# graehl/carmel

Hardware: AMD Instinct MI355X
Metric: arc-updates/sec (EM iterations/sec x derivation-lattice arcs swept per iteration) (higher is better)
Workload: dtype f64; 1 GPU; c4: synthetic 1000000-state / 9999990-arc WFST, 1000000 training pairs per GPU (random walks of 5-40 arcs), conditional normalisation, cached lattices; parallelism=corpus-sharded x1, none

## Files before the change

### carmel_amd/_capi.py

```python
import ctypes as C
import os

import numpy as np

_HERE = os.path.dirname(os.path.abspath(__file__))
LIB_PATH = os.environ.get("CARMEL_HIP_LIB") or os.path.join(_HERE, "libcarmel_hip.so")

SYMBOLS = [
    "carmel_hip_last_error", "carmel_hip_device_count", "carmel_hip_create", "carmel_hip_destroy",
    "carmel_hip_set_corpus", "carmel_hip_build_lattices", "carmel_hip_set_norm", "carmel_hip_set_prior",
    "carmel_hip_set_cascade", "carmel_hip_normalize", "carmel_hip_set_weights", "carmel_hip_get_weights",
    "carmel_hip_get_arc_weights", "carmel_hip_estimate", "carmel_hip_estimate_async",
    "carmel_hip_estimate_finish", "carmel_hip_counts_dev", "carmel_hip_counts_len", "carmel_hip_stream",
    "carmel_hip_use_external_counts", "carmel_hip_synchronize", "carmel_hip_last_sweep_ms", "carmel_hip_read_scalars",
    "carmel_hip_get_counts", "carmel_hip_set_counts", "carmel_hip_maximize", "carmel_hip_keep_em_weights", "carmel_hip_random_restart", "carmel_hip_save_counts",
    "carmel_hip_fractional_counts", "carmel_hip_set_digamma",
    "carmel_hip_save_best", "carmel_hip_load_best", "carmel_hip_host_build", "carmel_hip_host_dims",
    "carmel_hip_host_export", "carmel_hip_host_export_lanes", "carmel_hip_host_export_waves", "carmel_hip_host_transpose", "carmel_hip_host_tile_sweep", "carmel_hip_host_free",
    "carmel_hip_gibbs_create", "carmel_hip_gibbs_destroy", "carmel_hip_gibbs_n_blocks", "carmel_hip_gibbs_lattice_stats", "carmel_hip_gibbs_max_sample",
    "carmel_hip_gibbs_run", "carmel_hip_gibbs_run_ex", "carmel_hip_gibbs_set_prior_inference", "carmel_hip_gibbs_prior_trace",
    "carmel_hip_gibbs_n_prior_scales", "carmel_hip_gibbs_set_run_share", "carmel_hip_gibbs_best_stats", "carmel_hip_forests_set_prior_inference", "carmel_hip_forests_prior_trace", "carmel_hip_gibbs_get_sample", "carmel_hip_gibbs_set_observer", "carmel_hip_gibbs_current_probs", "carmel_hip_gibbs_get_state", "carmel_hip_gibbs_final_counts", "carmel_hip_gibbs_uniform", "carmel_hip_gibbs_power", "carmel_hip_gibbs_best_run", "carmel_hip_gibbs_set_init_weights",
    "carmel_hip_forests_create", "carmel_hip_forests_destroy", "carmel_hip_forests_estimate",
    "carmel_hip_forests_get_counts", "carmel_hip_forests_maximize", "carmel_hip_forests_get_weights",
    "carmel_hip_forests_set_weights", "carmel_hip_forests_set_alphas", "carmel_hip_forests_gibbs", "carmel_hip_forests_best_run", "carmel_hip_forests_final_counts", "carmel_hip_forests_get_sample",
    "carmel_hip_forests_max_sample", "carmel_hip_forests_viterbi", "carmel_hip_forests_get_viterbi",
    "carmel_hip_compose", "carmel_hip_composition_states", "carmel_hip_composition_arcs", "carmel_hip_composition_seconds",
    "carmel_hip_composition_export", "carmel_hip_composition_free",
    "carmel_hip_debug_lattice_fingerprint", "carmel_hip_lattice_layout", "carmel_hip_lattice_tile_sweep", "carmel_hip_lattice_fused_lanes", "carmel_hip_lattice_weight_source", "carmel_hip_accumulate_counts",
    "carmel_hip_comm_unique_id", "carmel_hip_comm_create", "carmel_hip_comm_destroy", "carmel_hip_comm_rank",
    "carmel_hip_comm_world", "carmel_hip_allreduce_counts", "carmel_hip_comm_allreduce_host",
    "carmel_hip_comm_abort", "carmel_hip_comm_transport_name", "carmel_hip_comm_create_custom", "carmel_hip_comm_set_sendrecv", "carmel_hip_comm_selftest", "carmel_hip_exchange_plan",
    "carmel_hip_exchange_info", "carmel_hip_exchange_measure", "carmel_hip_exchange_clear", "carmel_hip_set_layout_policy", "carmel_hip_set_matrix_fb",
    "carmel_hip_set_option", "carmel_hip_get_option", "carmel_hip_option_count", "carmel_hip_option_name",
    "carmel_hip_decoder_create", "carmel_hip_decoder_set_weights", "carmel_hip_decode", "carmel_hip_decoder_get_paths",
    "carmel_hip_decoder_last_ms", "carmel_hip_decoder_destroy",
    "carmel_hip_decode_kbest", "carmel_hip_decoder_kbest_size", "carmel_hip_decoder_get_kbest",
    "carmel_hip_decode_sum",
]


class LatticeStats(C.Structure):
    _fields_ = [(n, C.c_uint64) for n in (
        "n_pairs", "n_pairs_kept", "explored_states", "explored_arcs", "kept_states", "kept_arcs",
        "n_cyclic_pairs", "n_bundles", "max_levels", "device_bytes")] + [("build_seconds", C.c_double)] + [
            (n, C.c_uint64) for n in ("last_pair_explored_states", "last_pair_kept_states", "last_pair_kept_arcs",
                                      "n_windowed_pairs")]


class EstimateResult(C.Structure):
    _fields_ = [("sum_logprob", C.c_double), ("sum_weighted_logprob", C.c_double), ("n_pairs", C.c_uint64),
                ("kernel_ms", C.c_double)]


GIBBS_OBSERVER_FN = C.CFUNCTYPE(None, C.c_void_p, C.c_uint32, C.c_uint32, C.c_double)


class GibbsOpts(C.Structure):
    _fields_ = [("iter", C.c_uint32), ("burnin", C.c_uint32), ("seed", C.c_uint64), ("mode", C.c_int),
                ("uniform_p0", C.c_int), ("dirichlet_p0", C.c_int), ("final_counts", C.c_int),
                ("exclude_prior", C.c_int), ("min_prior", C.c_double), ("high_temp", C.c_double),
                ("low_temp", C.c_double), ("expectation", C.c_int), ("restarts", C.c_uint32), ("argmax_final", C.c_int),
                ("argmax_sum", C.c_int), ("include_self", C.c_int), ("random_start", C.c_int)]


def _load():
    if not os.path.exists(LIB_PATH):
        raise ImportError(
            "carmel_amd: %s not found — build it with `make -C carmel_amd/csrc` (or __graft_entry__.build()); "
            "there is no CPU fallback for the EM hot path" % LIB_PATH)
    lib = C.CDLL(LIB_PATH)
    for s in SYMBOLS:
        if not hasattr(lib, s):
            raise ImportError("carmel_amd: %s lacks symbol %s" % (LIB_PATH, s))
    lib.carmel_hip_last_error.restype = C.c_char_p
    lib.carmel_hip_counts_dev.restype = C.c_void_p
    lib.carmel_hip_stream.restype = C.c_void_p
    lib.carmel_hip_counts_len.restype = C.c_uint64
    vp = C.c_void_p
    lib.carmel_hip_last_error.argtypes = []
    lib.carmel_hip_device_count.argtypes = []
    lib.carmel_hip_set_option.argtypes = [C.c_char_p, C.c_char_p]
    lib.carmel_hip_get_option.argtypes = [C.c_char_p]
    lib.carmel_hip_get_option.restype = C.c_char_p
    lib.carmel_hip_option_count.argtypes = []
    lib.carmel_hip_option_name.argtypes = [C.c_int]
    lib.carmel_hip_option_name.restype = C.c_char_p
    lib.carmel_hip_random_restart.argtypes = [vp, C.c_uint64, C.c_uint32]
    lib.carmel_hip_keep_em_weights.argtypes = [vp]
    lib.carmel_hip_comm_unique_id.argtypes = [vp]
    lib.carmel_hip_debug_lattice_fingerprint.argtypes = [vp, vp]
    lib.carmel_hip_compose.argtypes = [C.POINTER(vp), C.c_int, C.c_uint32, vp, vp, vp, vp, vp, C.c_uint32, vp, vp, vp, vp, vp, vp,
                                       C.c_uint32, vp, C.c_uint32, C.c_uint32]
    lib.carmel_hip_composition_states.argtypes = [vp]
    lib.carmel_hip_composition_states.restype = C.c_uint64
    lib.carmel_hip_composition_arcs.argtypes = [vp]
    lib.carmel_hip_composition_arcs.restype = C.c_uint64
    lib.carmel_hip_composition_seconds.argtypes = [vp]
    lib.carmel_hip_composition_seconds.restype = C.c_double
    lib.carmel_hip_composition_export.argtypes = [vp] * 11
    lib.carmel_hip_composition_free.argtypes = [vp]
    lib.carmel_hip_comm_create.argtypes = [C.POINTER(vp), C.c_int, C.c_int, C.c_int, vp]
    lib.carmel_hip_comm_destroy.argtypes = [vp]
    lib.carmel_hip_comm_abort.argtypes = [vp]
    lib.carmel_hip_comm_transport_name.argtypes = [vp]
    lib.carmel_hip_comm_transport_name.restype = C.c_char_p
    lib.carmel_hip_comm_create_custom.argtypes = [C.POINTER(vp), C.c_int, C.c_int, C.c_int, vp]
    lib.carmel_hip_comm_set_sendrecv.argtypes = [vp, vp]
    lib.carmel_hip_comm_selftest.argtypes = [vp, C.c_uint32]
    lib.carmel_hip_exchange_plan.argtypes = [vp, vp, C.c_uint32, C.c_int]
    lib.carmel_hip_exchange_info.argtypes = [vp, C.POINTER(C.c_int), C.POINTER(C.c_uint32), C.POINTER(C.c_uint64), C.POINTER(C.c_uint64),
                                             C.POINTER(C.c_uint64)]
    lib.carmel_hip_exchange_measure.argtypes = [vp, C.c_uint32, C.POINTER(C.c_double)]
    lib.carmel_hip_exchange_clear.argtypes = [vp]
    lib.carmel_hip_set_layout_policy.argtypes = [vp, C.c_int]
    lib.carmel_hip_set_matrix_fb.argtypes = [vp, C.c_int]
    lib.carmel_hip_comm_rank.argtypes = [vp]
    lib.carmel_hip_comm_world.argtypes = [vp]
    lib.carmel_hip_allreduce_counts.argtypes = [vp, vp]
    lib.carmel_hip_comm_allreduce_host.argtypes = [vp, vp, C.c_uint32, C.c_int]
    lib.carmel_hip_fractional_counts.argtypes = [vp]
    lib.carmel_hip_set_digamma.argtypes = [vp, C.c_uint32, vp, vp]
    lib.carmel_hip_forests_set_alphas.argtypes = [vp, vp, C.c_uint32]
    lib.carmel_hip_create.argtypes = [C.POINTER(vp), C.c_int, C.c_uint32, C.c_uint32, C.c_uint64, vp, vp, vp, vp, vp, vp]
    lib.carmel_hip_destroy.argtypes = [vp]
    lib.carmel_hip_set_corpus.argtypes = [vp, C.c_uint64, vp, vp, vp, vp, vp]
    lib.carmel_hip_build_lattices.argtypes = [vp, C.c_int, C.c_int, vp, C.POINTER(LatticeStats)]
    lib.carmel_hip_set_norm.argtypes = [vp, C.c_int, C.c_double]
    lib.carmel_hip_set_prior.argtypes = [vp, C.c_double, C.c_int]
    lib.carmel_hip_set_cascade.argtypes = [vp, C.c_uint64, vp, vp, vp, vp, vp, C.c_uint32, vp, vp, C.c_uint64, vp, vp]
    lib.carmel_hip_normalize.argtypes = [vp]
    lib.carmel_hip_set_weights.argtypes = [vp, vp]
    lib.carmel_hip_get_weights.argtypes = [vp, vp]
    lib.carmel_hip_get_arc_weights.argtypes = [vp, vp]
    lib.carmel_hip_estimate.argtypes = [vp, C.POINTER(EstimateResult), vp]
    lib.carmel_hip_estimate_async.argtypes = [vp]
    lib.carmel_hip_estimate_finish.argtypes = [vp, C.POINTER(EstimateResult), vp]
    lib.carmel_hip_counts_dev.argtypes = [vp]
    lib.carmel_hip_counts_len.argtypes = [vp]
    lib.carmel_hip_stream.argtypes = [vp]
    lib.carmel_hip_use_external_counts.argtypes = [vp, vp]
    lib.carmel_hip_synchronize.argtypes = [vp]
    lib.carmel_hip_last_sweep_ms.argtypes = [vp, C.POINTER(C.c_double)]
    lib.carmel_hip_read_scalars.argtypes = [vp, C.POINTER(EstimateResult)]
    lib.carmel_hip_get_counts.argtypes = [vp, vp]
    lib.carmel_hip_set_counts.argtypes = [vp, vp]
    lib.carmel_hip_maximize.argtypes = [vp, C.c_double, C.POINTER(C.c_double)]
    lib.carmel_hip_save_counts.argtypes = [vp]
    lib.carmel_hip_save_best.argtypes = [vp]
    lib.carmel_hip_load_best.argtypes = [vp]
    lib.carmel_hip_host_build.argtypes = [C.POINTER(vp), C.c_uint32, C.c_uint32, C.c_uint64, vp, vp, vp, vp,
                                          C.c_uint64, vp, vp, vp, vp, vp, C.c_int, C.c_int, C.c_uint32, C.c_uint32,
                                          C.c_int]
    lib.carmel_hip_host_dims.argtypes = [vp, vp]
    lib.carmel_hip_host_dims.restype = None
    lib.carmel_hip_host_export.argtypes = [vp] + [vp] * 12
    lib.carmel_hip_host_export.restype = None
    lib.carmel_hip_host_export_lanes.argtypes = [vp] * 8
    lib.carmel_hip_host_export_waves.argtypes = [vp] * 10
    lib.carmel_hip_host_transpose.argtypes = [vp] * 12
    lib.carmel_hip_host_transpose.restype = None
    lib.carmel_hip_host_tile_sweep.argtypes = [vp] * 3
    lib.carmel_hip_host_tile_sweep.restype = None
    lib.carmel_hip_host_export_lanes.restype = None
    lib.carmel_hip_host_free.argtypes = [vp]
    lib.carmel_hip_host_free.restype = None
    lib.carmel_hip_gibbs_create.argtypes = [C.POINTER(vp), vp, C.POINTER(GibbsOpts)]
    lib.carmel_hip_gibbs_destroy.argtypes = [vp]
    lib.carmel_hip_gibbs_n_blocks.argtypes = [vp]
    lib.carmel_hip_gibbs_lattice_stats.argtypes = [vp, C.POINTER(LatticeStats)]
    lib.carmel_hip_gibbs_n_blocks.restype = C.c_uint32
    lib.carmel_hip_gibbs_max_sample.argtypes = [vp]
    lib.carmel_hip_gibbs_max_sample.restype = C.c_uint32
    lib.carmel_hip_gibbs_set_init_weights.argtypes = [vp, vp]
    lib.carmel_hip_gibbs_best_run.argtypes = [vp]
    lib.carmel_hip_gibbs_best_run.restype = C.c_uint32
    lib.carmel_hip_gibbs_run.argtypes = [vp, vp, vp]
    lib.carmel_hip_gibbs_run_ex.argtypes = [vp, vp, vp, vp]
    lib.carmel_hip_gibbs_set_prior_inference.argtypes = [vp, C.c_double, C.c_int, C.c_int, C.c_int, C.c_uint32, C.c_uint32, vp, vp, C.c_uint32]
    lib.carmel_hip_gibbs_prior_trace.argtypes = [vp, vp, C.c_uint32, vp, C.c_uint32]
    lib.carmel_hip_gibbs_n_prior_scales.argtypes = [vp]
    lib.carmel_hip_gibbs_set_run_share.argtypes = [vp, C.c_uint32, C.c_uint32]
    lib.carmel_hip_gibbs_best_stats.argtypes = [vp, vp, vp]
    lib.carmel_hip_lattice_layout.argtypes = [vp]
    lib.carmel_hip_lattice_tile_sweep.argtypes = [vp]
    lib.carmel_hip_lattice_fused_lanes.argtypes = [vp]
    lib.carmel_hip_lattice_weight_source.argtypes = [vp]
    lib.carmel_hip_accumulate_counts.argtypes = [vp, C.c_int]
    lib.carmel_hip_forests_set_prior_inference.argtypes = [vp, C.c_double, C.c_int, C.c_int, C.c_uint32, C.c_uint32]
    lib.carmel_hip_forests_prior_trace.argtypes = [vp, vp, C.c_uint32, vp, C.c_uint32, vp]
    lib.carmel_hip_gibbs_n_prior_scales.restype = C.c_uint32
    lib.carmel_hip_gibbs_get_sample.argtypes = [vp, C.c_uint32, vp, C.POINTER(C.c_uint32)]
    lib.carmel_hip_gibbs_set_observer.argtypes = [vp, C.c_uint32, GIBBS_OBSERVER_FN, vp]
    lib.carmel_hip_gibbs_current_probs.argtypes = [vp, vp]
    lib.carmel_hip_gibbs_get_state.argtypes = [vp, vp, vp, vp, vp, vp]
    lib.carmel_hip_gibbs_final_counts.argtypes = [vp, vp]
    lib.carmel_hip_gibbs_uniform.argtypes = [C.c_uint64, C.c_uint32, C.c_uint32, C.c_uint32]
    lib.carmel_hip_gibbs_uniform.restype = C.c_double
    lib.carmel_hip_gibbs_power.argtypes = [C.c_double, C.c_double, C.c_uint32, C.c_uint32]
    lib.carmel_hip_gibbs_power.restype = C.c_double
    lib.carmel_hip_forests_create.argtypes = [C.POINTER(vp), C.c_int, C.c_uint64, vp, vp, vp, vp, C.c_uint32, vp,
                                              C.c_uint64, vp, vp]
    lib.carmel_hip_forests_destroy.argtypes = [vp]
    lib.carmel_hip_forests_estimate.argtypes = [vp, C.c_double, C.POINTER(C.c_double), C.POINTER(C.c_uint64), vp]
    lib.carmel_hip_forests_get_counts.argtypes = [vp, C.c_double, vp]
    lib.carmel_hip_forests_maximize.argtypes = [vp, C.c_double, C.c_double, C.c_int, C.POINTER(C.c_double)]
    lib.carmel_hip_forests_get_weights.argtypes = [vp, vp]
    lib.carmel_hip_forests_set_weights.argtypes = [vp, vp]
    lib.carmel_hip_forests_gibbs.argtypes = [vp, C.POINTER(GibbsOpts), C.c_double, vp, vp]
    lib.carmel_hip_forests_best_run.argtypes = [vp]
    lib.carmel_hip_forests_best_run.restype = C.c_uint32
    lib.carmel_hip_forests_final_counts.argtypes = [vp, vp]
    lib.carmel_hip_forests_get_sample.argtypes = [vp, C.c_uint64, vp, C.POINTER(C.c_uint32)]
    lib.carmel_hip_forests_max_sample.argtypes = [vp]
    lib.carmel_hip_forests_max_sample.restype = C.c_uint32
    lib.carmel_hip_forests_viterbi.argtypes = [vp, vp]
    lib.carmel_hip_forests_get_viterbi.argtypes = [vp, C.c_uint64, vp, vp, C.POINTER(C.c_uint32)]
    lib.carmel_hip_decoder_create.argtypes = [C.POINTER(vp), C.c_int, C.c_uint32, C.c_uint32, C.c_uint64, vp, vp, vp, vp, vp,
                                              C.c_int]
    lib.carmel_hip_decoder_set_weights.argtypes = [vp, vp]
    lib.carmel_hip_decode.argtypes = [vp, C.c_uint64, vp, vp, vp, vp]
    lib.carmel_hip_decoder_get_paths.argtypes = [vp, vp]
    lib.carmel_hip_decoder_last_ms.argtypes = [vp, C.POINTER(C.c_double)]
    lib.carmel_hip_decoder_destroy.argtypes = [vp]
    lib.carmel_hip_decode_kbest.argtypes = [vp, C.c_uint32, C.c_uint64, vp, vp, vp]
    lib.carmel_hip_decoder_kbest_size.argtypes = [vp, C.POINTER(C.c_uint64), C.POINTER(C.c_uint64)]
    lib.carmel_hip_decoder_get_kbest.argtypes = [vp, vp, vp, vp]
    lib.carmel_hip_decode_sum.argtypes = [vp, C.c_uint64, vp, vp, vp]
    for s in SYMBOLS:
        if getattr(lib, s).argtypes is None:
            raise ImportError("carmel_amd: no ctypes prototype for %s" % s)
    return lib


lib = _load()


class CarmelHipError(RuntimeError):
    def __init__(self, code, where):
        self.code = code
        RuntimeError.__init__(self, "%s failed (%d): %s" % (where, code, lib.carmel_hip_last_error().decode()))


def check(rc, where):
    if rc != 0:
        raise CarmelHipError(rc, where)


def set_option(key, value):
    rc = lib.carmel_hip_set_option(key.encode(), None if value is None else str(value).encode())
    if rc != 0:
        raise ValueError("libcarmel_hip has no option %r (it has: %s)" % (key, ", ".join(option_names())))


def get_option(key):
    v = lib.carmel_hip_get_option(key.encode())
    return None if v is None else v.decode()


def option_names():
    return [lib.carmel_hip_option_name(i).decode() for i in range(lib.carmel_hip_option_count())]


def options_from_env(environ=None):
    names = set(option_names())
    for k, v in (os.environ if environ is None else environ).items():
        key = "timing" if k == "CARMEL_TIMING" else k[len("CARMEL_HIP_"):].lower() if k.startswith("CARMEL_HIP_") and k != "CARMEL_HIP_LIB" else None
        if key in names:
            set_option(key, v)


def ptr(a):
    if a is None:
        return None
    assert a.flags["C_CONTIGUOUS"]
    return a.ctypes.data_as(C.c_void_p)


def u32(a):
    return np.ascontiguousarray(a, dtype=np.uint32)


def u64(a):
    return np.ascontiguousarray(a, dtype=np.uint64)


def f64(a):
    return np.ascontiguousarray(a, dtype=np.float64)
```

### carmel_amd/csrc/engine.cpp

```cpp
#include <hip/hip_runtime.h>
#include <chrono>
#include <cmath>
#include <cstdio>
#include <cstring>
#include <cstdlib>
#include <limits>
#include <string>
#include <thread>
#include <unordered_map>
#include <vector>
#include "engine.hpp"
#include "options.hpp"
#include "host/refhash.hpp"
#include "rng.hpp"
#include "unrolled_args.hpp"

int unrolled_try_build(carmel_hip_trainer* t, int host_threads, uint8_t* has_derivation, carmel_hip_lattice_stats* stats);
int gpu_build_lattices(carmel_hip_trainer* t, const BuildOptions& opt, uint8_t* has_derivation, carmel_hip_lattice_stats* stats,
                       bool& done);
int gpu_tables_for_host_layout(carmel_hip_trainer* t, const std::vector<uint32_t>& lane_arc, const std::vector<uint32_t>& wave_arc);
int carmel_hip_debug_lattice_fingerprint_impl(carmel_hip_trainer* t, uint64_t* out);
int build_run_tables(carmel_hip_trainer* t);
int exchange_weights_in(carmel_hip_trainer* t, ExchangePlan* xp, const TransArgs& T, bool need_x);
int exchange_counts_out(carmel_hip_trainer* t, ExchangePlan* xp, const TransArgs& T);
int exchange_counts_tail(carmel_hip_trainer* t, ExchangePlan* xp);
int exchange_maximize(carmel_hip_trainer* t, ExchangePlan* xp, double* max_change, int* handled);
int exchange_settle(carmel_hip_trainer* t, bool need_counts);
void exchange_drop(carmel_hip_trainer* t);
int unrolled_estimate(carmel_hip_trainer* t, hipStream_t s);

static thread_local std::string g_err;
namespace carmel_hip {
int fail(int code, const std::string& msg) {
  g_err = msg;
  return code;
}
}

template <class F>
static void host_parallel_for(size_t n, F f) {
  const size_t nt = n < (1u << 20) ? 1 : std::min<size_t>(16, std::max<unsigned>(1, std::thread::hardware_concurrency()));
  if (nt <= 1) {
    f(0, n);
    return;
  }
  std::vector<std::thread> th;
  for (size_t k = 0; k < nt; ++k) th.emplace_back([&, k]() { f(n * k / nt, n * (k + 1) / nt); });
  for (auto& x : th) x.join();
}

extern "C" {

const char* carmel_hip_last_error(void) { return g_err.c_str(); }

int carmel_hip_device_count(void) {
  int n = 0;
  if (hipGetDeviceCount(&n) != hipSuccess) return 0;
  return n;
}

int carmel_hip_create(carmel_hip_trainer** out, int device, uint32_t n_states, uint32_t final_state, uint64_t n_arcs,
                      const uint32_t* src, const uint32_t* dst, const uint32_t* in_sym, const uint32_t* out_sym,
                      const double* logw, const uint32_t* group) {
  if (!out || !src || !dst || !in_sym || !out_sym || !logw) return fail(CARMEL_HIP_ERR_ARG, "null argument");
  if (final_state >= n_states) return fail(CARMEL_HIP_ERR_ARG, "final state out of range");
  if (n_arcs >= 0xfffffff0ull) return fail(CARMEL_HIP_ERR_ARG, "arc ids are 32-bit (derivations.h GraphArc data)");
  int ndev = 0;
  HIPCHK(hipGetDeviceCount(&ndev));
  if (ndev <= 0) return fail(CARMEL_HIP_ERR_HIP, "no HIP device: the EM hot path has no CPU fallback");
  if (device < 0 || device >= ndev) return fail(CARMEL_HIP_ERR_ARG, "bad device index");
  HIPCHK(hipSetDevice(device));
  carmel_hip_trainer* t = new carmel_hip_trainer();
  t->device = device;
  hipError_t e = hipStreamCreateWithFlags(&t->stream, hipStreamNonBlocking);
  if (e != hipSuccess) {
    delete t;
    return fail(CARMEL_HIP_ERR_HIP, hipGetErrorString(e));
  }
  (void)hipEventCreate(&t->ev0);
  (void)hipEventCreate(&t->ev1);
  (void)hipStreamCreateWithFlags(&t->side, hipStreamNonBlocking);
  (void)hipEventCreateWithFlags(&t->ev_fork, hipEventDisableTiming);
  (void)hipEventCreateWithFlags(&t->ev_join, hipEventDisableTiming);
  (void)hipEventCreateWithFlags(&t->ev_w, hipEventDisableTiming);
  if (hipHostMalloc((void**)&t->h_box, 2 * sizeof(unsigned long long), hipHostMallocCoherent | hipHostMallocMapped) != hipSuccess) t->h_box = nullptr;
  if (t->h_box) t->h_box[0] = t->h_box[1] = 0;
  (void)hipStreamCreateWithFlags(&t->bstream, hipStreamNonBlocking);
  (void)hipEventCreateWithFlags(&t->ev_b0, hipEventDisableTiming);
  (void)hipEventCreateWithFlags(&t->ev_b1, hipEventDisableTiming);
  for (int k = 0; k < carmel_hip_trainer::N_CHUNK_STREAMS; ++k) {
    (void)hipStreamCreateWithFlags(&t->cstream[k], hipStreamNonBlocking);
    (void)hipEventCreateWithFlags(&t->cev[k], hipEventDisableTiming);
  }
  HostWfst& w = t->w;
  w.n_states = n_states;
  w.final_state = final_state;
  w.n_arcs = n_arcs;
  w.src.assign(src, src + n_arcs);
  w.dst.assign(dst, dst + n_arcs);
  w.in.assign(in_sym, in_sym + n_arcs);
  w.out.assign(out_sym, out_sym + n_arcs);
  if (group)
    w.group.assign(group, group + n_arcs);
  else
    w.group.assign(n_arcs, CARMEL_HIP_NO_GROUP);
  for (uint64_t k = 0; k < n_arcs; ++k) {
    if (src[k] >= n_states || dst[k] >= n_states) {
      delete t;
      return fail(CARMEL_HIP_ERR_ARG, "arc endpoint out of range");
    }
    if (k && src[k] < src[k - 1]) {
      delete t;
      return fail(CARMEL_HIP_ERR_ARG, "arcs must be in arc-id order (state-major)");
    }
  }
  w.build_index();
  std::vector<double> lw(logw, logw + n_arcs);
  e = t->arc_logw.upload(lw, t->stream);
  if (e == hipSuccess) e = t->arc_group.upload(w.group, t->stream);
  if (e == hipSuccess) e = t->counts.alloc(n_arcs + 4);
  if (e == hipSuccess) e = t->old_logw.alloc(n_arcs);
  if (e == hipSuccess) e = t->em_logw.alloc(n_arcs);
  if (e == hipSuccess) e = t->best_logw.alloc(n_arcs);
  if (e == hipSuccess) e = t->maxchg.alloc(1);
  if (e == hipSuccess) e = hipStreamSynchronize(t->stream);
  if (e != hipSuccess) {
    delete t;
    return fail(CARMEL_HIP_ERR_HIP, hipGetErrorString(e));
  }
  *out = t;
  return CARMEL_HIP_OK;
}

int carmel_hip_destroy(carmel_hip_trainer* t) {
  if (t && t->xplan) exchange_drop(t);
  if (!t) return CARMEL_HIP_OK;
  (void)hipSetDevice(t->device);
  if (t->stream) (void)hipStreamSynchronize(t->stream);
  if (t->matrix) matrix_release(t->matrix);
  t->matrix = nullptr;
  if (t->ev0) (void)hipEventDestroy(t->ev0);
  if (t->ev1) (void)hipEventDestroy(t->ev1);
  if (t->side) (void)hipStreamSynchronize(t->side);
  if (t->ev_fork) (void)hipEventDestroy(t->ev_fork);
  if (t->ev_join) (void)hipEventDestroy(t->ev_join);
  if (t->ev_w) (void)hipEventDestroy(t->ev_w);
  if (t->h_box) (void)hipHostFree(t->h_box);
  if (t->bstream) {
    (void)hipStreamSynchronize(t->bstream);
    (void)hipStreamDestroy(t->bstream);
  }
  if (t->ev_b0) (void)hipEventDestroy(t->ev_b0);
  if (t->ev_b1) (void)hipEventDestroy(t->ev_b1);
  for (int k = 0; k < carmel_hip_trainer::N_CHUNK_STREAMS; ++k) {
    if (t->cstream[k]) {
      (void)hipStreamSynchronize(t->cstream[k]);
      (void)hipStreamDestroy(t->cstream[k]);
    }
    if (t->cev[k]) (void)hipEventDestroy(t->cev[k]);
    if (k == 0) {
      for (hipEvent_t e : t->ev_piece)
        if (e) (void)hipEventDestroy(e);
      t->ev_piece.clear();
    }
  }
// ... 17 lines not shown
    c.weight.assign(pair_weight, pair_weight + n_pairs);
  else
    c.weight.assign(n_pairs, 1.0);
  t->have_corpus = true;
  t->have_lattices = false;
  return CARMEL_HIP_OK;
}

int carmel_hip_build_lattices(carmel_hip_trainer* t, int prune, int host_threads, uint8_t* has_derivation,
                              carmel_hip_lattice_stats* stats) {
  if (!t) return fail(CARMEL_HIP_ERR_ARG, "null trainer");
  if (!t->have_corpus) return fail(CARMEL_HIP_ERR_STATE, "set_corpus first");
  HIPCHK(hipSetDevice(t->device));
  if (t->xplan) exchange_drop(t);
  if (t->scalars_pending) {
    (void)hipStreamSynchronize(t->side);
    t->scalars_pending = false;
  }
  t->build_prune = prune;
  t->build_threads = host_threads;
  if (t->matrix) {
    HIPCHK(hipStreamSynchronize(t->stream));
    matrix_release(t->matrix);
    t->matrix = nullptr;
  }
  {
    int rc = unrolled_try_build(t, host_threads, has_derivation, stats);
    if (rc) return rc;
    if (t->unrolled) return CARMEL_HIP_OK;
  }
  auto t0 = std::chrono::steady_clock::now();
  BuildOptions opt;
  opt.prune = prune != 0;
  opt.threads = host_threads;
  if (const char* e = lib_opt("lane_states")) opt.lane_states = (uint32_t)atoi(e);
  if (const char* e = lib_opt("tile_sweep")) opt.tile_sweep = atoi(e) != 0;
  if (const char* e = lib_opt("lane_fused")) opt.lane_fused = atoi(e) != 0;
  if (lib_opt("transpose") && atoi(lib_opt("transpose")) == 0) opt.lane_fused = false;
  if (const char* e = lib_opt("lane_chunks")) opt.lane_chunks = (uint32_t)std::max(1, atoi(e));
  if (const char* e = lib_opt("lane_window")) opt.lane_window = (uint32_t)std::max(0, atoi(e));
  if (const char* e = lib_opt("lane_window_min")) opt.lane_window_min = (uint32_t)std::max(0, atoi(e));
  if (const char* e = lib_opt("wave_ring")) opt.wave_ring = atoi(e) != 0;
  if (const char* e = lib_opt("wave_min_width")) opt.wave_min_width = opt.wave_lane_min_width = atof(e);
  {
    const bool want_gpu = !(lib_opt("gpu_build") && atoi(lib_opt("gpu_build")) == 0) &&
                          !(lib_opt("transpose") && atoi(lib_opt("transpose")) == 0);
    bool probe_ok = true;
    if (want_gpu && t->corpus.n_pairs > 4096) {
      const uint64_t np = t->corpus.n_pairs, n_probe = 64;
      for (uint64_t k = 0; k < n_probe && probe_ok; ++k) {
        const uint64_t p = k * (np / n_probe);
        PairLattice pl;
        bool hd = false;
        build_pair_lattice(t->w, t->corpus.in_sym.data() + t->corpus.in_off[p], (uint32_t)(t->corpus.in_off[p + 1] - t->corpus.in_off[p]),
                           t->corpus.out_sym.data() + t->corpus.out_off[p], (uint32_t)(t->corpus.out_off[p + 1] - t->corpus.out_off[p]),
                           opt.prune, pl, hd);
        if (pl.explored_states > 200 || (hd && (pl.n_states > opt.lane_states || pl.edges.size() > 200))) opt.gpu_large_caps = true;
        if (pl.explored_states > 1024 || (hd && (pl.cyclic || pl.n_states > 1023 || pl.edges.size() > 1536))) probe_ok = false;
      }
    }
    if (want_gpu && probe_ok) {
      bool done = false;
      int rc = gpu_build_lattices(t, opt, has_derivation, stats, done);
      if (rc) return rc;
      if (!done && !opt.gpu_large_caps) {
        opt.gpu_large_caps = true;
        rc = gpu_build_lattices(t, opt, has_derivation, stats, done);
        if (rc) return rc;
        if (!done) opt.gpu_large_caps = false;
      }
      if (done) {
        if (lib_opt("timing")) fprintf(stderr, "timing: lattices built on the GPU\n");
        rc = build_run_tables(t);
        if (stats) stats->device_bytes = t->device_bytes;
        return rc;
      }
    }
  }
  std::string err;
  LatticeSet& L = t->lat;
  L = LatticeSet();
  {
    const char* e = lib_opt("wave_gather");
    const bool want_t = !(lib_opt("transpose") && atoi(lib_opt("transpose")) == 0);
    opt.wave_gather = want_t && (e ? atoi(e) != 0 : t->w.n_arcs * sizeof(double) <= (128ull << 20));
  }
  opt.device_tables = !(lib_opt("transpose") && atoi(lib_opt("transpose")) == 0) &&
                      !(lib_opt("device_tables") && atoi(lib_opt("device_tables")) == 0);
  if (!build_lattices(t->w, t->corpus, opt, L, err)) return fail(CARMEL_HIP_ERR_ARG, err);
  const bool have_tables = !L.t_buckets.empty() || L.tables_deferred;
  if (has_derivation) std::memcpy(has_derivation, L.has_deriv.data(), L.has_deriv.size());
  hipStream_t s = t->stream;
  HIPCHK(t->bundles.upload(L.bundles, s));
  HIPCHK(t->in_arcs.upload(L.in_arcs, s));
  HIPCHK(t->out_arcs.upload(L.out_arcs, s));
  HIPCHK(t->in_off.upload(L.in_off, s));
  HIPCHK(t->out_off.upload(L.out_off, s));
  HIPCHK(t->level_off.upload(L.level_off, s));
  HIPCHK(t->pair_start.upload(L.pair_start, s));
  HIPCHK(t->pair_final.upload(L.pair_final, s));
  HIPCHK(t->pair_id.upload(L.pair_id, s));
  HIPCHK(t->pair_logw.upload(L.pair_logw, s));
  HIPCHK(t->lane_groups.upload(L.lane_groups, s));
  if (L.tile_sweep)
    HIPCHK(t->tile_group.upload(L.tile_group, s));
  else
    t->tile_group.release();
  HIPCHK(t->wave_descs.upload(L.waves, s));
  HIPCHK(t->wave_fwd.upload(L.wave_fwd, s));
  HIPCHK(t->wave_bwd.upload(L.wave_bwd, s));
  if (L.wave_gather && !L.waves.empty())
    HIPCHK(t->wave_bwd_arc.upload(L.wave_bwd_arc, s));
  else
    t->wave_bwd_arc.release();
  HIPCHK(t->wave_level_off.upload(L.wave_level_off, s));
  HIPCHK(t->wave_frow.upload(L.wave_frow, s));
  HIPCHK(t->wave_brow.upload(L.wave_brow, s));
  t->wave_slot_base = L.wave_slot_base;
  t->wave_records = L.wave_bwd.size();
  HIPCHK(t->wave_spill.alloc(L.wave_spill_states));
  {
    const bool want_t = !(lib_opt("transpose") && atoi(lib_opt("transpose")) == 0);
    if (want_t && have_tables) {
      std::vector<uint32_t> fx(L.lane_fwd.size());
      host_parallel_for(fx.size(), [&](size_t k0, size_t k1) {
        for (size_t k = k0; k < k1; ++k) fx[k] = L.lane_fwd[k].x;
      });
      HIPCHK(t->lane_fwdx.upload(fx, s));
      HIPCHK(hipStreamSynchronize(s));
      t->lane_fwd.release();
    } else {
      HIPCHK(t->lane_fwd.upload(L.lane_fwd, s));
      t->lane_fwdx.release();
    }
  }
  {
    std::vector<uint32_t> bx(L.lane_bwd.size());
    host_parallel_for(bx.size(), [&](size_t k0, size_t k1) {
      for (size_t k = k0; k < k1; ++k) bx[k] = L.lane_bwd[k].x;
    });
    HIPCHK(t->lane_bwd.upload(bx, s));
    HIPCHK(hipStreamSynchronize(s));
  }
  HIPCHK(t->lane_pair.upload(L.lane_pair, s));
  HIPCHK(t->lane_nstates.upload(L.lane_nstates, s));
  HIPCHK(t->lane_logw.upload(L.lane_logw, s));
  if (L.tile_sweep && t->lane_fwdx.n) {
    HIPCHK(t->lane_rec2.alloc(t->lane_bwd.n));
    HIPCHK(t->lane_chain.alloc(t->lane_groups.n));
    HIPCHK(t->tile_chain.alloc(t->tile_group.n - 1));
    HIPCHK(hipMemsetAsync(t->lane_rec2.p, 0, t->lane_rec2.bytes(), s));
    HIPCHK(launch_pack_tile_records(t->lane_groups.p, (uint32_t)t->lane_groups.n, t->lane_nstates.p, t->lane_fwdx.p, t->lane_bwd.p, t->lane_rec2.p, t->lane_chain.p,
                                    t->tile_group.p, (uint32_t)(t->tile_group.n - 1), t->tile_chain.p, s));
    if (lib_opt("timing")) {
      std::vector<uint32_t> ch(t->lane_chain.n);
      HIPCHK(hipMemcpyAsync(ch.data(), t->lane_chain.p, ch.size() * 4, hipMemcpyDeviceToHost, s));
      HIPCHK(hipStreamSynchronize(s));
      size_t n1 = 0;
      for (uint32_t c : ch) n1 += c & 1u;
      fprintf(stderr, "timing: tile sweep: %zu tiles, %zu groups, %zu of them single paths\n", L.tile_group.size() - 1, ch.size(), n1);
    }
  } else {
    t->lane_rec2.release();
    t->lane_chain.release();
    t->tile_chain.release();
  }
  t->lane_records = L.wave_slot_base + L.wave_bwd.size();
  if (L.lane_fused)
    t->post.release();
  else
    HIPCHK(t->post.alloc(L.n_post));
  HIPCHK(t->wcache.alloc(t->wave_bwd_arc.n ? L.wave_slot_base : t->lane_records));
  if (!L.waves.empty() && !have_tables)
    return fail(CARMEL_HIP_ERR_UNSUPPORTED, "lattice set too large for the blocked transposition (2^32 items) with one-per-wavefront lattices");
  if (L.lane_spill_rows)
    HIPCHK(t->lane_spill.alloc(L.lane_spill_rows * 64));
  else
    t->lane_spill.release();
  if (L.tables_deferred) {
    std::vector<uint32_t> la(L.lane_bwd.size());
    host_parallel_for(la.size(), [&](size_t k0, size_t k1) {
      for (size_t k = k0; k < k1; ++k) la[k] = (L.lane_bwd[k].x & LANE_VALID) ? L.lane_bwd[k].y : 0xffffffffu;
    });
    t->hot_chunks.release();
    int rc = gpu_tables_for_host_layout(t, la, L.wave_bwd_arc);
    if (rc) return rc;
    t->use_transpose = true;
  } else {
    HIPCHK(t->arc_off.upload(L.arc_off, s));
    HIPCHK(t->slot_pos.upload(L.slot_pos, s));
    HIPCHK(t->hot_chunks.upload(L.hot_chunks, s));
    {
      const bool want = !(lib_opt("transpose") && atoi(lib_opt("transpose")) == 0);
      t->use_transpose = want && !L.t_buckets.empty();
      if (t->use_transpose) {
        HIPCHK(t->t_buckets.upload(L.t_buckets, s));
        HIPCHK(t->t_tile_base.upload(L.t_tile_base, s));
        HIPCHK(t->t_b_arc.upload(L.t_b_arc, s));
        HIPCHK(t->t_b_rank.upload(L.t_b_rank, s));
        HIPCHK(t->t_b_src.upload(L.t_b_src, s));
        HIPCHK(t->t_t_pos.upload(L.t_t_pos, s));
        HIPCHK(t->t_t_src.upload(L.t_t_src, s));
        HIPCHK(t->t_a_off.upload(L.t_a_off, s));
        HIPCHK(t->t_split_arcs.upload(L.t_split_arcs, s));
        HIPCHK(t->t_x.alloc(L.slot_pos.size()));
        HIPCHK(t->t_xc.alloc(L.slot_pos.size()));
        HIPCHK(hipStreamSynchronize(s));
      }
      std::vector<uint16_t>().swap(L.t_b_arc);
      std::vector<uint16_t>().swap(L.t_a_off);
      std::vector<uint16_t>().swap(L.t_b_rank);
      std::vector<uint16_t>().swap(L.t_t_pos);
      std::vector<uint32_t>().swap(L.t_b_src);
      std::vector<uint32_t>().swap(L.t_t_src);
    }
  }
  if (!L.waves.empty() && !t->use_transpose)
    return fail(CARMEL_HIP_ERR_UNSUPPORTED, "one-per-wavefront lattices need the blocked transposition (CARMEL_HIP_TRANSPOSE=0 is for lane corpora)");
  HIPCHK(t->pair_logprob.alloc(t->corpus.n_pairs));
  {
    std::vector<double> pw(t->corpus.n_pairs);
    for (uint64_t p = 0; p < t->corpus.n_pairs; ++p)
      pw[p] = L.has_deriv[p] ? (t->corpus.weight.empty() ? 1.0 : t->corpus.weight[p]) : -1.0;
    HIPCHK(t->pair_w.upload(pw, s));
    HIPCHK(t->scalar_partial.alloc(3 * 256));
    HIPCHK(hipStreamSynchronize(s));
  }
  bool need_val = false, need_val2 = false;
  for (auto& lc : L.classes) {
    if (lc.serial || lc.max_states == 0) need_val = true;
    if (lc.serial) need_val2 = true;
  }
  HIPCHK(t->alpha_g.alloc(need_val ? L.in_off.size() : 0));
  HIPCHK(t->beta_g.alloc(need_val2 ? L.in_off.size() : 0));
  HIPCHK(launch_fill(t->pair_logprob.p, -std::numeric_limits<double>::infinity(), t->corpus.n_pairs, s));
  HIPCHK(hipStreamSynchronize(s));
  t->device_bytes = t->bundles.bytes() + t->in_arcs.bytes() + t->out_arcs.bytes() + t->in_off.bytes() +
                    t->out_off.bytes() + t->level_off.bytes() + t->pair_start.bytes() + t->pair_final.bytes() +
                    t->pair_id.bytes() + t->pair_logw.bytes() + t->pair_logprob.bytes() + t->alpha_g.bytes() +
                    t->beta_g.bytes() + t->lane_groups.bytes() + t->lane_fwd.bytes() + t->lane_fwdx.bytes() + t->lane_bwd.bytes() +
                    t->lane_pair.bytes() + t->lane_nstates.bytes() + t->lane_logw.bytes() + t->post.bytes() + t->wcache.bytes() +
                    t->arc_off.bytes() + t->slot_pos.bytes() + t->hot_chunks.bytes() + t->t_b_arc.bytes() + t->t_b_rank.bytes() +
                    t->t_t_pos.bytes() + t->t_b_src.bytes() + t->t_t_src.bytes() + t->t_x.bytes() + t->t_xc.bytes() +
                    t->wave_descs.bytes() + t->wave_fwd.bytes() + t->wave_bwd.bytes() + t->wave_bwd_arc.bytes() + t->wave_level_off.bytes() +
                    t->wave_frow.bytes() + t->wave_brow.bytes() + t->wave_spill.bytes();
  std::vector<uint64_t>().swap(L.arc_off);
  std::vector<uint64_t>().swap(L.slot_pos);
  std::vector<uint2_t>().swap(L.lane_fwd);
  std::vector<uint2_t>().swap(L.lane_bwd);
  std::vector<uint2_t>().swap(L.wave_fwd);
  std::vector<uint32_t>().swap(L.wave_bwd);
  std::vector<uint32_t>().swap(L.wave_bwd_arc);
  std::vector<uint2_t>().swap(L.in_arcs);
  std::vector<uint2_t>().swap(L.out_arcs);
  std::vector<uint32_t>().swap(L.in_off);
  std::vector<uint32_t>().swap(L.out_off);
  std::vector<uint32_t>().swap(L.level_off);
  if (lib_opt("timing")) {
    fprintf(stderr, "timing: layout lane_arcs=%llu lane_groups=%zu lane_pieces=%zu bundles=%zu bundle_classes=%zu total_arcs=%llu aligned=%d\n",
            (unsigned long long)L.lane_arcs, L.lane_groups.size(), L.lane_classes.size(), L.bundles.size(), L.classes.size(),
            (unsigned long long)L.total_arcs, (int)L.lane_tiles_aligned);
    for (auto& lc : L.lane_classes) fprintf(stderr, "timing:   lane piece groups=%u %s=%u tiles=%u\n", lc.count, lc.windowed ? "window" : "max_states", lc.max_states, lc.tile_count);
    for (auto& wc : L.wave_classes) fprintf(stderr, "timing:   wave class count=%u max_states=%u max_width=%u ring=%u\n", wc.count, wc.max_states, wc.max_width, wc.ring);
    for (auto& lc : L.classes) fprintf(stderr, "timing:   bundle class count=%u block=%u max_states=%u serial=%d\n", lc.count, lc.block, lc.max_states, (int)lc.serial);
  }
  t->have_lattices = true;
  ++t->lattice_epoch;
  {
    int rc = build_run_tables(t);
    if (rc) return rc;
  }
  if (stats) {
    stats->n_pairs = t->corpus.n_pairs;
    stats->n_pairs_kept = L.n_kept;
    stats->explored_states = L.explored_states;
    stats->explored_arcs = L.explored_arcs;
    stats->kept_states = L.total_states;
    stats->kept_arcs = L.total_arcs;
    stats->n_cyclic_pairs = L.n_cyclic;
    stats->n_bundles = L.bundles.size() + L.lane_groups.size() + L.waves.size();
    stats->max_levels = L.max_levels;
    stats->device_bytes = t->device_bytes;
    stats->build_seconds = std::chrono::duration<double>(std::chrono::steady_clock::now() - t0).count();
    stats->last_pair_explored_states = L.last_pre_states;
    stats->last_pair_kept_states = L.last_post_states;
    stats->last_pair_kept_arcs = L.last_post_arcs;
    stats->n_windowed_pairs = 0;
    for (auto& g : L.lane_groups)
      if (g.window) stats->n_windowed_pairs += g.n_lanes;
  }
  return CARMEL_HIP_OK;
}

static int build_ties(carmel_hip_trainer* t, uint64_t n, const uint32_t* member, const uint32_t* group) {
  std::vector<uint32_t> tie_of(n, 0xffffffffu);
  std::unordered_map<uint64_t, uint32_t> ids;
  t->any_locked = false;
  t->h_tie_member.clear();
  for (uint64_t k = 0; k < n; ++k) {
    if (group[k] == CARMEL_HIP_LOCKED_GROUP) t->any_locked = true;
    if (group[k] == CARMEL_HIP_NO_GROUP || group[k] == CARMEL_HIP_LOCKED_GROUP) continue;
    const uint64_t key = ((uint64_t)(member ? member[k] : 0) << 32) | group[k];
    auto it = ids.find(key);
    if (it == ids.end()) {
      it = ids.emplace(key, (uint32_t)ids.size()).first;
      t->h_tie_member.push_back(member ? member[k] : 0);
    }
    tie_of[k] = it->second;
  }
  t->n_ties = ids.size();
  if (t->n_ties) {
    HIPCHK(t->tie_of.upload(tie_of, t->stream));
    HIPCHK(t->tie_tab.alloc(4 * t->n_ties));
    HIPCHK(hipStreamSynchronize(t->stream));
  } else {
    t->tie_of.release();
    t->tie_tab.release();
  }
// ... 488 lines not shown
  A.out_arcs = (const uint2*)t->out_arcs.p;
  A.in_off = t->in_off.p;
  A.out_off = t->out_off.p;
  A.level_off = t->level_off.p;
  A.pair_start = t->pair_start.p;
  A.pair_final = t->pair_final.p;
  A.pair_id = t->pair_id.p;
  A.pair_logw = t->pair_logw.p;
  A.logw = t->arc_logw.p;
  A.post = t->post.p + t->lane_records;
  A.scalars = t->counts_ptr() + t->w.n_arcs;
  A.pair_logprob = t->pair_logprob.p;
  A.val_g = t->alpha_g.p;
  A.val2_g = t->beta_g.p;
  A.first_bundle = 0;
  LaneArgs LA;
  LA.groups = t->lane_groups.p;
  LA.fwd = (const uint2*)t->lane_fwd.p;
  LA.fwdx = t->lane_fwdx.p;
  LA.bwd = t->lane_bwd.p;
  LA.rec2 = t->lane_rec2.p;
  LA.chain = t->lane_chain.p;
  LA.tile_chain = t->tile_chain.p;
  LA.lane_pair = t->lane_pair.p;
  LA.lane_nstates = t->lane_nstates.p;
  LA.lane_logw = t->lane_logw.p;
  LA.logw = t->arc_logw.p;
  LA.post = t->post.p;
  LA.wcache = t->wcache.p;
  LA.scalars = t->counts_ptr() + t->w.n_arcs;
  LA.pair_logprob = t->pair_logprob.p;
  LA.spill = t->lane_spill.p;
  LA.first_group = 0;
  LA.lds_rows = 0;
  LA.xc_tile_base = nullptr;
  LA.xc_t_pos = nullptr;
  LA.xc = nullptr;
  LA.trace = nullptr;
  const char* trace_path = lib_opt("lane_trace");
  static DevBuf<unsigned long long> trace_buf;
  if (trace_path) {
    if (trace_buf.n != t->lane_groups.n * 16) {
      HIPCHK(trace_buf.alloc(t->lane_groups.n * 16));
      HIPCHK(hipMemset(trace_buf.p, 0, trace_buf.bytes()));
    }
    LA.trace = trace_buf.p;
  }
  WaveArgs WA;
  WA.descs = t->wave_descs.p;
  WA.fwd = (const uint2*)t->wave_fwd.p;
  WA.bwd = t->wave_bwd.p;
  WA.level_off = t->wave_level_off.p;
  WA.frow = t->wave_frow.p;
  WA.brow = t->wave_brow.p;
  WA.wcache = t->wcache.p + t->wave_slot_base;
  if (t->wave_bwd_arc.n) {
    WA.wcache = nullptr;
    WA.logw = t->arc_logw.p;
    WA.bwd_arc = t->wave_bwd_arc.p;
    WA.n_arcs = (uint32_t)t->w.n_arcs;
  }
  WA.post = t->post.p + t->wave_slot_base;
  WA.pair_logprob = t->pair_logprob.p;
  WA.spill = t->wave_spill.p;
  WA.first = 0;
  WA.max_states = WA.max_width = 0;
  TransArgs T;
  trans_args(t, T);
  const bool wave_xc = t->use_transpose && t->wave_xc_idx.n && !T.use_runs && !(T.scatter & 2u);
  if (wave_xc) {
    WA.xc = T.xc;
    WA.xc_idx = t->wave_xc_idx.p;
  }
  LA.pre_weights = t->use_transpose ? 1u : 0u;
  const bool lane_fused = t->use_transpose && t->lat.lane_fused &&
                          !(lib_opt("lane_fused_kernel") && atoi(lib_opt("lane_fused_kernel")) == 0);
  if (lane_fused) {
    LA.xc_tile_base = T.tile_base;
    LA.xc_t_pos = T.t_pos;
    LA.xc = T.xc;
  } else if (t->lat.lane_fused && !t->post.n && t->lat.n_post) {
    HIPCHK(t->post.alloc(t->lat.n_post));
    T.post = LA.post = t->post.p;
    T.n_post = t->post.n;
  }
  ExchangePlan* const xp = (t->xplan && exchange_is_sharded(t->xplan) && t->use_transpose) ? t->xplan : nullptr;
  if (timed) HIPCHK(hipEventRecord(t->ev0, s));
  const uint32_t lane_tiles = (uint32_t)((t->wcache.n + t->lat.tile - 1) / t->lat.tile);
  const bool tile_kernel_off = lib_opt("tile_sweep_kernel") && atoi(lib_opt("tile_sweep_kernel")) == 0;
  const bool tile_sweep = t->use_transpose && t->lat.tile_sweep && t->tile_group.n && !tile_kernel_off &&
                          ((T.scatter & 3u) == 0u || ((T.scatter & 3u) == 3u && T.use_runs));
  bool tile_sweep_done = false;
  const bool tile_gather = t->use_transpose && t->t_t_arc.n && !T.use_runs && !(T.scatter & 1u);
  TransArgs TW = T;
  if (tile_gather) {
    TW.x = const_cast<double*>(T.logw);
    TW.t_src = t->t_t_arc.p;
  }
  TransArgs TZ = TW;
  if (!xp) {
    TZ.zero_list = t->t_split_arcs.p;
    TZ.n_zero = (uint32_t)t->t_split_arcs.n;
  }
  const bool side_by_side = t->use_transpose && t->lat.lane_classes.size() > 1 && t->lat.lane_tiles_aligned && t->lat.wave_classes.empty();
  const bool bundles_beside = side_by_side && !t->lat.classes.empty();
  if (xp) {
    int rc = exchange_weights_in(t, xp, T, t->wcache.n && !tile_gather);
    if (rc) return rc;
  } else if (t->use_transpose && t->wcache.n && !tile_gather)
    HIPCHK(launch_trans_w_bucket(T, s));
  if (bundles_beside) {
    HIPCHK(hipEventRecord(t->ev_b0, s));
    HIPCHK(hipStreamWaitEvent(t->bstream, t->ev_b0, 0));
    for (auto& lc : t->lat.classes) HIPCHK(launch_sweep(A, lc, t->bstream));
    HIPCHK(hipEventRecord(t->ev_b1, t->bstream));
  }
  if (side_by_side && t->lat.lane_fused) {
    HIPCHK(hipEventRecord(t->ev_w, s));
    hipStream_t ps = t->side, ss = s;
    HIPCHK(hipStreamWaitEvent(ps, t->ev_w, 0));
    const size_t np = t->lat.lane_classes.size();
    while (t->ev_piece.size() < np) {
      hipEvent_t e = nullptr;
      HIPCHK(hipEventCreateWithFlags(&e, hipEventDisableTiming));
      t->ev_piece.push_back(e);
    }
    for (size_t k = 0; k < np; ++k) {
      const auto& lc = t->lat.lane_classes[k];
      HIPCHK(launch_trans_w_tiles(TW, lc.tile_first, lc.tile_count, ps));
      HIPCHK(hipEventRecord(t->ev_piece[k], ps));
      HIPCHK(hipStreamWaitEvent(ss, t->ev_piece[k], 0));
      HIPCHK(launch_lane_sweep(LA, lc, ss, lane_fused));
      if (!lane_fused) HIPCHK(launch_trans_c_tiles(T, lc.tile_first, lc.tile_count, ss));
    }
  } else if (side_by_side) {
    HIPCHK(hipEventRecord(t->ev_w, s));
    const int NS = carmel_hip_trainer::N_CHUNK_STREAMS;
    bool used[carmel_hip_trainer::N_CHUNK_STREAMS] = {false, false, false, false};
    size_t k = 0;
    for (auto& lc : t->lat.lane_classes) {
      hipStream_t cs = t->cstream[k % NS];
      if (!used[k % NS]) HIPCHK(hipStreamWaitEvent(cs, t->ev_w, 0));
      used[k % NS] = true;
      HIPCHK(launch_trans_w_tiles(TW, lc.tile_first, lc.tile_count, cs));
      HIPCHK(launch_lane_sweep(LA, lc, cs, lane_fused));
      if (!lane_fused) HIPCHK(launch_trans_c_tiles(T, lc.tile_first, lc.tile_count, cs));
      ++k;
    }
    for (int q = 0; q < NS; ++q)
      if (used[q]) {
        HIPCHK(hipEventRecord(t->cev[q], t->cstream[q]));
        HIPCHK(hipStreamWaitEvent(s, t->cev[q], 0));
      }
  } else if (tile_sweep && launch_tile_sweep(TZ, LA, t->tile_group.p, 0, lane_tiles, s) == hipSuccess) {
    tile_sweep_done = true;
  } else {
    if (tile_sweep) (void)hipGetLastError();
    if (t->use_transpose) HIPCHK(launch_trans_w_tiles(TW, 0, lane_tiles, s));
    if (t->lat.wave_classes.size() > 1 || (!t->lat.wave_classes.empty() && !t->lat.lane_classes.empty())) {
      HIPCHK(hipEventRecord(t->ev_w, s));
      const int NS = carmel_hip_trainer::N_CHUNK_STREAMS;
      bool used[carmel_hip_trainer::N_CHUNK_STREAMS] = {false, false, false, false};
      size_t k = 0;
      for (auto& wc : t->lat.wave_classes) {
        hipStream_t cs = t->cstream[k % NS];
        if (!used[k % NS]) HIPCHK(hipStreamWaitEvent(cs, t->ev_w, 0));
        used[k % NS] = true;
        HIPCHK(launch_wave_sweep(WA, wc, cs));
        ++k;
      }
      for (auto& lc : t->lat.lane_classes) HIPCHK(launch_lane_sweep(LA, lc, s, lane_fused));
      for (int q = 0; q < NS; ++q)
        if (used[q]) {
          HIPCHK(hipEventRecord(t->cev[q], t->cstream[q]));
          HIPCHK(hipStreamWaitEvent(s, t->cev[q], 0));
        }
    } else {
      for (auto& wc : t->lat.wave_classes) HIPCHK(launch_wave_sweep(WA, wc, s));
      for (auto& lc : t->lat.lane_classes) HIPCHK(launch_lane_sweep(LA, lc, s, lane_fused));
    }
  }
  if (bundles_beside)
    HIPCHK(hipStreamWaitEvent(s, t->ev_b1, 0));
  else
    for (auto& lc : t->lat.classes) HIPCHK(launch_sweep(A, lc, s));
  ReduceArgs R;
  R.arc_off = t->arc_off.p;
  R.slot_pos = t->slot_pos.p;
  R.hot_chunks = t->hot_chunks.p;
  R.post = t->post.p;
  R.counts = t->counts_ptr();
  R.n_arcs = t->w.n_arcs;
  R.n_hot_chunks = t->hot_chunks.n / 3;
  auto fork_scalars = [&](hipEvent_t fork) -> int {
    HIPCHK(hipEventRecord(fork, s));
    HIPCHK(hipStreamWaitEvent(t->side, fork, 0));
    HIPCHK(launch_scalars(t->pair_logprob.p, t->pair_w.p, t->corpus.n_pairs, t->scalar_partial.p,
                          t->counts_ptr() + t->w.n_arcs, t->side));
    HIPCHK(hipEventRecord(t->ev_join, t->side));
    t->scalars_pending = true;
    return CARMEL_HIP_OK;
  };
  if (xp) {
    int rc = fork_scalars(t->ev_fork);
    if (rc) return rc;
  }
  if (t->use_transpose) {
    const uint32_t first = (side_by_side || tile_sweep_done || lane_fused) ? lane_tiles : 0u;
    const uint32_t end = wave_xc ? std::min(T.n_tiles, (uint32_t)(t->wave_slot_base / t->lat.tile)) : T.n_tiles;
    HIPCHK(launch_trans_c_tiles(T, first, end > first ? end - first : 0u, s));
    if (xp) {
      int rc = exchange_counts_out(t, xp, T);
      if (rc) return rc;
    } else if (tile_sweep_done)
      HIPCHK(launch_trans_c_bucket_range(T, 0, T.n_buckets, s));
    else
      HIPCHK(launch_trans_c_bucket(T, t->t_split_arcs.p, (uint32_t)t->t_split_arcs.n, s));
  } else
    HIPCHK(launch_count_reduce(R, s));
  if (xp) {
    if (timed) HIPCHK(hipEventRecord(t->ev1, s));
  } else {
    int rc = fork_scalars(timed ? t->ev1 : t->ev_fork);
    if (rc) return rc;
  }
  if (xp || t->ext_counts) {
    int rc = scalars_join(t);
    if (rc) return rc;
  }
  if (xp) {
    int rc = exchange_counts_tail(t, xp);
    if (rc) return rc;
  }
  if (timed && trace_path && trace_buf.n) {
    std::vector<unsigned long long> h(trace_buf.n);
    HIPCHK(hipStreamSynchronize(s));
    HIPCHK(hipMemcpy(h.data(), trace_buf.p, h.size() * 8, hipMemcpyDeviceToHost));
    if (FILE* f = fopen(trace_path, "wb")) {
      fwrite(h.data(), 8, h.size(), f);
      fclose(f);
    }
  }
  return CARMEL_HIP_OK;
}

int carmel_hip_estimate_async(carmel_hip_trainer* t) {
  if (!t) return fail(CARMEL_HIP_ERR_ARG, "null trainer");
  if (!t->have_lattices) return fail(CARMEL_HIP_ERR_STATE, "build_lattices first");
  HIPCHK(hipSetDevice(t->device));
  return estimate_enqueue(t, true);
}

int carmel_hip_set_layout_policy(carmel_hip_trainer* t, int allow_unrolled) {
  if (!t) return fail(CARMEL_HIP_ERR_ARG, "null trainer");
  t->allow_unrolled = allow_unrolled != 0;
  return CARMEL_HIP_OK;
}
int carmel_hip_set_matrix_fb(carmel_hip_trainer* t, int on) {
  if (!t) return fail(CARMEL_HIP_ERR_ARG, "null trainer");
  HIPCHK(hipSetDevice(t->device));
  if (t->matrix) {
    HIPCHK(hipStreamSynchronize(t->stream));
    matrix_release(t->matrix);
    t->matrix = nullptr;
  }
  if (!on) return CARMEL_HIP_OK;
  if (!t->have_lattices) return fail(CARMEL_HIP_ERR_STATE, "carmel_hip_set_matrix_fb: build_lattices first (it finds the pairs without a derivation)");
  if (t->xplan) return fail(CARMEL_HIP_ERR_STATE, "carmel_hip_set_matrix_fb: drop the exchange plan first (the matrix E-step keeps the one all-reduce)");
  if (t->unrolled) {
    const bool keep = t->allow_unrolled;
    t->allow_unrolled = false;
    const int rc = carmel_hip_build_lattices(t, t->build_prune, t->build_threads, nullptr, nullptr);
    t->allow_unrolled = keep;
    if (rc) return rc;
  }
  return matrix_setup(t, &t->matrix);
}
int carmel_hip_lattice_tile_sweep(carmel_hip_trainer* t) {
  if (!t || !t->have_lattices || t->unrolled || !t->lat.tile_sweep || !t->tile_group.n) return 0;
  return (int)(t->tile_group.n - 1);
}
int carmel_hip_lattice_fused_lanes(carmel_hip_trainer* t) {
  if (!t || !t->have_lattices || t->unrolled || !t->use_transpose || !t->lat.lane_fused) return 0;
  return (int)((t->wcache.n + t->lat.tile - 1) / t->lat.tile);
}
int carmel_hip_lattice_weight_source(carmel_hip_trainer* t) {
  if (!t || !t->have_lattices || t->unrolled || !t->use_transpose) return 0;
  return (t->t_t_arc.n ? 1 : 0) | (t->wave_bwd_arc.n ? 2 : 0) | (t->wave_xc_idx.n ? 4 : 0);
}
int carmel_hip_lattice_layout(carmel_hip_trainer* t) {
  if (!t || !t->have_lattices) return -1;
  return t->unrolled ? (t->dense ? 2 : 1) : 0;
}

int carmel_hip_read_scalars(carmel_hip_trainer* t, carmel_hip_estimate_result* res) {
  if (!t || !res) return fail(CARMEL_HIP_ERR_ARG, "null argument");
  HIPCHK(hipSetDevice(t->device));
  if (t->xplan) {
    int xrc = exchange_settle(t, false);
    if (xrc) return xrc;
  }
  int jrc = scalars_join(t);
  if (jrc) return jrc;
  double sc[4];
  HIPCHK(hipMemcpyAsync(sc, t->counts_ptr() + t->w.n_arcs, sizeof sc, hipMemcpyDeviceToHost, t->stream));
  HIPCHK(hipStreamSynchronize(t->stream));
  res->sum_logprob = sc[0];
  res->sum_weighted_logprob = sc[1];
  res->n_pairs = (uint64_t)(sc[2] + 0.5);
  return CARMEL_HIP_OK;
}

int carmel_hip_estimate_finish(carmel_hip_trainer* t, carmel_hip_estimate_result* res, double* per_pair_logprob) {
  if (!t) return fail(CARMEL_HIP_ERR_ARG, "null trainer");
  HIPCHK(hipSetDevice(t->device));
  carmel_hip_estimate_result r;
  std::memset(&r, 0, sizeof r);
  int rc = carmel_hip_read_scalars(t, &r);
  if (rc) return rc;
  float ms = 0;
  HIPCHK(hipEventElapsedTime(&ms, t->ev0, t->ev1));
  r.kernel_ms = ms;
  if (per_pair_logprob) {
    HIPCHK(hipMemcpyAsync(per_pair_logprob, t->pair_logprob.p, t->corpus.n_pairs * sizeof(double),
                          hipMemcpyDeviceToHost, t->stream));
    HIPCHK(hipStreamSynchronize(t->stream));
  }
  if (res) *res = r;
  if ((t->unrolled ? t->um.pair_id.size() : t->lat.n_kept) == 0)
    return fail(CARMEL_HIP_ERR_NO_DERIV, "No training example had a derivation - aborting training.");
  return CARMEL_HIP_OK;
}

int carmel_hip_estimate(carmel_hip_trainer* t, carmel_hip_estimate_result* res, double* per_pair_logprob) {
  int rc = carmel_hip_estimate_async(t);
  if (rc) return rc;
  return carmel_hip_estimate_finish(t, res, per_pair_logprob);
}

void* carmel_hip_counts_dev(carmel_hip_trainer* t) { return t ? (void*)t->counts_ptr() : nullptr; }
int carmel_hip_use_external_counts(carmel_hip_trainer* t, void* dev_ptr) {
  if (!t) return fail(CARMEL_HIP_ERR_ARG, "null trainer");
  if (dev_ptr && t->xplan && exchange_is_sharded(t->xplan))
    return fail(CARMEL_HIP_ERR_STATE, "carmel_hip_use_external_counts: a sharded exchange is planned -- carmel_hip_exchange_clear (collective) "
                                      "or destroy / abort the communicator first");
  t->ext_counts = (double*)dev_ptr;
  return CARMEL_HIP_OK;
}
int carmel_hip_last_sweep_ms(carmel_hip_trainer* t, double* ms) {
  if (!t || !ms) return fail(CARMEL_HIP_ERR_ARG, "null argument");
  HIPCHK(hipSetDevice(t->device));
  HIPCHK(hipEventSynchronize(t->ev1));
  float f = 0;
  HIPCHK(hipEventElapsedTime(&f, t->ev0, t->ev1));
  *ms = f;
  return CARMEL_HIP_OK;
}
int carmel_hip_synchronize(carmel_hip_trainer* t) {
  if (!t) return fail(CARMEL_HIP_ERR_ARG, "null trainer");
  HIPCHK(hipSetDevice(t->device));
  if (t->xplan) {
    int xrc = exchange_settle(t, false);
    if (xrc) return xrc;
  }
  int jrc = scalars_join(t);
  if (jrc) return jrc;
  HIPCHK(hipStreamSynchronize(t->stream));
  return CARMEL_HIP_OK;
}
uint64_t carmel_hip_counts_len(carmel_hip_trainer* t) { return t ? t->w.n_arcs + 4 : 0; }
void* carmel_hip_stream(carmel_hip_trainer* t) { return t ? (void*)t->stream : nullptr; }

int carmel_hip_get_counts(carmel_hip_trainer* t, double* counts) {
  if (!t || !counts) return fail(CARMEL_HIP_ERR_ARG, "null argument");
  HIPCHK(hipSetDevice(t->device));
  if (t->unrolled && t->cascade) {
    const double need = (double)t->um.lattice_arcs * 64.0;
    size_t free_b = 0, total_b = 0;
    HIPCHK(hipMemGetInfo(&free_b, &total_b));
    if (t->um.lattice_arcs >= (1ull << 31) || need > 0.5 * (double)free_b)
      return fail(CARMEL_HIP_ERR_UNSUPPORTED, "composed-arc counts under the unrolled sweep need explicit lattices: " +
                                                  std::to_string((unsigned long long)(need / 1e9)) + " GB for this corpus");
    std::vector<double> aw(t->w.n_arcs);
    HIPCHK(hipMemcpyAsync(aw.data(), t->arc_logw.p, aw.size() * sizeof(double), hipMemcpyDeviceToHost, t->stream));
    HIPCHK(hipStreamSynchronize(t->stream));
    carmel_hip_trainer* x = nullptr;
    int rc = carmel_hip_create(&x, t->device, t->w.n_states, t->w.final_state, t->w.n_arcs, t->w.src.data(), t->w.dst.data(),
                               t->w.in.data(), t->w.out.data(), aw.data(), nullptr);
    if (rc) return rc;
    struct Guard {
      carmel_hip_trainer* x;
      ~Guard() { carmel_hip_destroy(x); }
    } guard{x};
    x->allow_unrolled = false;
    const HostCorpus& c = t->corpus;
    rc = carmel_hip_set_corpus(x, c.n_pairs, c.in_off.data(), c.in_sym.data(), c.out_off.data(), c.out_sym.data(),
                               c.weight.empty() ? nullptr : c.weight.data());
    if (!rc) rc = carmel_hip_build_lattices(x, 1, 0, nullptr, nullptr);
    carmel_hip_estimate_result er;
    if (!rc) rc = carmel_hip_estimate(x, &er, nullptr);
    if (rc) return rc;
    HIPCHK(hipMemcpyAsync(counts, x->counts_ptr(), t->w.n_arcs * sizeof(double), hipMemcpyDeviceToHost, x->stream));
    HIPCHK(hipStreamSynchronize(x->stream));
    return CARMEL_HIP_OK;
  }
  if (t->xplan) {
    int xrc = exchange_settle(t, true);
    if (xrc) return xrc;
  }
  HIPCHK(hipMemcpyAsync(counts, t->counts_ptr(), t->w.n_arcs * sizeof(double), hipMemcpyDeviceToHost, t->stream));
  HIPCHK(hipStreamSynchronize(t->stream));
  return CARMEL_HIP_OK;
}
int carmel_hip_set_counts(carmel_hip_trainer* t, const double* counts) {
  if (!t || !counts) return fail(CARMEL_HIP_ERR_ARG, "null argument");
  HIPCHK(hipSetDevice(t->device));
  if (t->xplan) {
    int xrc = exchange_settle(t, false);
    if (xrc) return xrc;
  }
  HIPCHK(hipMemcpyAsync(t->counts_ptr(), counts, t->w.n_arcs * sizeof(double), hipMemcpyHostToDevice, t->stream));
  HIPCHK(hipStreamSynchronize(t->stream));
  return CARMEL_HIP_OK;
}

int carmel_hip_accumulate_counts(carmel_hip_trainer* t, int op) {
  if (!t) return fail(CARMEL_HIP_ERR_ARG, "null trainer");
  HIPCHK(hipSetDevice(t->device));
  if (t->xplan) return fail(CARMEL_HIP_ERR_STATE, "carmel_hip_accumulate_counts: drop the exchange plan first (its pieces follow one lattice set's buckets)");
// ... 243 lines not shown
```

### carmel_amd/csrc/engine.hpp

```cpp
#pragma once
#include <hip/hip_runtime.h>
#include <cstdlib>
#include <string>
#include <vector>
#include "../../include/carmel_hip.h"
#include "options.hpp"
#include "kernels.hpp"
#include "unrolled_args.hpp"

namespace carmel_hip {
int fail(int code, const std::string& msg);
}
using carmel_hip::fail;
using namespace carmel_hip;

#define HIPCHK(x)                                                                                             \
  do {                                                                                                        \
    hipError_t e_ = (x);                                                                                      \
    if (e_ != hipSuccess)                                                                                     \
      return fail(CARMEL_HIP_ERR_HIP, std::string(#x) + ": " + hipGetErrorString(e_));                        \
  } while (0)

static const size_t DEVBUF_SLACK = 131072;
template <class T>
struct DevBuf {
  T* p = nullptr;
  size_t n = 0;
  ~DevBuf() { release(); }
  void release() {
    if (p) (void)hipFree(p);
    p = nullptr;
    n = 0;
  }
  hipError_t alloc(size_t count) {
    release();
    n = count;
    if (!count) return hipSuccess;
    hipError_t e = hipMalloc((void**)&p, count * sizeof(T) + DEVBUF_SLACK);
    const bool poison = lib_opt("poison") && atoi(lib_opt("poison"));
    if (poison && e == hipSuccess) {
      e = hipMemset(p, 0xff, count * sizeof(T) + DEVBUF_SLACK);
      if (e == hipSuccess) e = hipDeviceSynchronize();
    }
    return e;
  }
  hipError_t upload(const std::vector<T>& v, hipStream_t s) {
    hipError_t e = alloc(v.size());
    if (e != hipSuccess || v.empty()) return e;
    return hipMemcpyAsync(p, v.data(), v.size() * sizeof(T), hipMemcpyHostToDevice, s);
  }
  size_t bytes() const { return n * sizeof(T); }
};

struct ExchangePlan;
struct carmel_hip_trainer {
  ExchangePlan* xplan = nullptr;
  int device = 0;
  hipStream_t stream = nullptr;
  hipEvent_t ev0 = nullptr, ev1 = nullptr;
  hipStream_t side = nullptr;
  hipEvent_t ev_fork = nullptr, ev_join = nullptr;
  static const int N_CHUNK_STREAMS = 4;
  hipStream_t cstream[N_CHUNK_STREAMS] = {nullptr, nullptr, nullptr, nullptr};
  hipEvent_t cev[N_CHUNK_STREAMS] = {nullptr, nullptr, nullptr, nullptr};
  std::vector<hipEvent_t> ev_piece;
  hipEvent_t ev_w = nullptr;
  hipStream_t bstream = nullptr;
  hipEvent_t ev_b0 = nullptr, ev_b1 = nullptr;
  HostWfst w;
  HostCorpus corpus;
  bool have_corpus = false, have_lattices = false, cascade = false;
  LatticeSet lat;
  DevBuf<double> arc_logw;
  DevBuf<double> counts;
  DevBuf<uint32_t> arc_group;
  DevBuf<double> param_logw_c, param_counts_c;
  DevBuf<uint32_t> param_group_c;
  DevBuf<uint64_t> chain_off, chain_param;
  uint64_t n_params = 0, n_chains = 0;
  DevBuf<double> old_logw, em_logw, best_logw, prior;
  DevBuf<double> mstep_snap;
  bool any_locked = false;
  DevBuf<uint32_t> norm_of;
  DevBuf<uint16_t> norm_code16;
  DevBuf<uint32_t> norm_mask32, norm_lockmask32;
  DevBuf<unsigned long long> norm_mask64, norm_lockmask64;
  DevBuf<uint32_t> tie_of;
  DevBuf<double> glocked;
  DevBuf<double> tie_tab;
  uint64_t n_ties = 0;
  DevBuf<uint64_t> group_off, norm_perm, big_groups;
  DevBuf<double> add_count, gscale;
  DevBuf<double> dig_alpha, tie_alpha;
  bool any_digamma = false;
  std::vector<uint32_t> h_group_member, h_tie_member;
  std::vector<uint32_t> h_group_src;
  std::vector<uint8_t> h_group_joint;
  std::vector<uint32_t> h_group_ref_rank;
  DevBuf<double> arc_prior_w;
  std::vector<double> h_arc_prior_w;
  DevBuf<double> u_param_wprior;
  bool any_add_count = false;
  DevBuf<unsigned long long> maxchg;
  unsigned long long* h_box = nullptr;
  unsigned long long box_seq = 0;
  bool scalars_pending = false;
  uint64_t n_norm_groups = 0;
  bool have_norm = false, have_prior = false, prior_nonzero = false;
  int norm_group_by = CARMEL_HIP_NORM_CONDITIONAL;
  double norm_add_count = 0, smooth_floor = 0;
  DevBuf<BundleDesc> bundles;
  DevBuf<uint2_t> in_arcs, out_arcs;
  DevBuf<uint32_t> in_off, out_off, level_off, pair_start, pair_final, pair_id;
  DevBuf<double> pair_logw, pair_logprob, alpha_g, beta_g;
  DevBuf<WaveDesc> wave_descs;
  DevBuf<uint2_t> wave_fwd;
  DevBuf<uint32_t> wave_xc_idx;
  DevBuf<uint32_t> wave_bwd_arc;
  DevBuf<uint32_t> wave_bwd, wave_level_off, wave_frow, wave_brow;
  uint64_t wave_slot_base = 0, wave_records = 0;
  DevBuf<double> wave_spill;
  DevBuf<LaneGroup> lane_groups;
  DevBuf<uint32_t> tile_group;
  DevBuf<uint32_t> lane_rec2;
  DevBuf<uint32_t> lane_chain;
  DevBuf<uint32_t> tile_chain;
  DevBuf<uint2_t> lane_fwd;
  DevBuf<TransBucket> t_buckets;
  DevBuf<uint64_t> t_tile_base;
  DevBuf<uint16_t> t_b_arc, t_b_rank, t_t_pos, t_a_off;
  DevBuf<uint32_t> t_b_src, t_t_src, t_split_arcs;
  DevBuf<uint32_t> t_t_arc;
  DevBuf<double> t_x, t_xc;
  DevBuf<uint32_t> tr_off, tr_src, br_off, br_src;
  DevBuf<uint16_t> tr_rel, br_rel;
  bool use_runs = false;
  DevBuf<unsigned long long> max_partial;
  uint32_t norm_span = 0;
  bool all_grouped = true;
  DevBuf<double> pair_w;
  DevBuf<double> scalar_partial;
  bool unrolled = false;
  bool allow_unrolled = true;
  UnrolledModel um;
  DevBuf<uint32_t> u_f_off, u_b_off, u_f_arc, u_b_arc, u_e_arc, u_pair_id;
  DevBuf<uint16_t> u_e_src, u_e_dst;
  DevBuf<uint32_t> u_slot_of;
  DevBuf<URec> u_f_rec, u_b_rec;
  DevBuf<uint16_t> u_e_slot, u_seq_sym;
  DevBuf<uint64_t> u_seq_off;
  DevBuf<double> u_We, u_pair_weight, u_partial, u_scratch;
  DevBuf<double> u_param_uses;
  DevBuf<double> u_em_param, u_best_param;
  uint32_t u_n_slots = 0, u_n_wg = 0;
  bool dense = false;
  uint32_t d_SP = 0, d_groups = 0;
  DevBuf<double> d_A, d_AT, d_B, d_vbuf, d_zbuf, d_afbuf, d_weight, d_partial;
  DevBuf<uint32_t> d_a_off, d_a_par, d_b_off, d_b_par, d_len, d_pair;
  DevBuf<uint8_t> d_a_has, d_b_has;
  DevBuf<uint16_t> d_Bslot, d_sym;
  DevBuf<uint64_t> d_sym_off, d_vbuf_off;
  uint64_t lattice_epoch = 0;
  bool use_transpose = false;
  bool em_valid = false;
  bool mstep_stream_work = false;
  DevBuf<uint32_t> lane_bwd;
  DevBuf<uint32_t> lane_fwdx;
  DevBuf<uint32_t> lane_pair, lane_nstates;
  DevBuf<double> lane_logw, post, wcache, lane_spill;
  DevBuf<double> counts_acc;
  DevBuf<uint64_t> arc_off, slot_pos, hot_chunks;
  uint64_t lane_records = 0;
  uint64_t device_bytes = 0;
  std::vector<uint32_t> h_norm_of, h_param_group;
  std::vector<uint64_t> h_group_off, h_norm_perm;
  std::vector<double> h_group_add;
  std::vector<uint64_t> h_chain_off, h_chain_param;

  int build_prune = 1, build_threads = 0;
  void* matrix = nullptr;
  double* ext_counts = nullptr;
  double* counts_ptr() { return ext_counts ? ext_counts : counts.p; }
  double* params() { return cascade ? param_logw_c.p : arc_logw.p; }
  double* pcounts() { return cascade ? param_counts_c.p : counts_ptr(); }
  uint32_t* pgroup() { return cascade ? param_group_c.p : arc_group.p; }
  uint64_t np() const { return cascade ? n_params : w.n_arcs; }
};

extern "C" int mstep_args(carmel_hip_trainer* t, int use_counts, int save_old, MstepArgs& M);
extern "C" void trans_args(carmel_hip_trainer* t, TransArgs& T);
bool exchange_is_sharded(const ExchangePlan* xp);
extern "C" int publish_u64(carmel_hip_trainer* t, const unsigned long long* dev, hipStream_t s);
extern "C" int fetch_u64(carmel_hip_trainer* t, const unsigned long long* dev, unsigned long long* out, hipStream_t s, bool published);
extern "C" int scalars_join(carmel_hip_trainer* t);
namespace carmel_hip {
int matrix_setup(carmel_hip_trainer* t, void** out);
int matrix_estimate(carmel_hip_trainer* t, void* state, hipStream_t s);
void matrix_release(void* state);
}
```

### carmel_amd/csrc/kernels.hpp

```cpp
#pragma once
#include <hip/hip_runtime.h>
#include <stdint.h>
#include "lattice.hpp"

namespace carmel_hip {

struct LaneArgs {
  const LaneGroup* groups;
  const uint2* fwd;
  const uint32_t* fwdx;
  const uint32_t* bwd;
  const uint32_t* rec2;
  const uint32_t* chain;
  const uint32_t* tile_chain;
  const uint32_t* lane_pair;
  const uint32_t* lane_nstates;
  const double* lane_logw;
  const double* logw;
  double* post;
  double* wcache;
  double* scalars;
  double* pair_logprob;
  double* spill;
  uint32_t first_group;
  uint32_t pre_weights;
  unsigned long long* trace;
  uint32_t lds_rows;
  const uint64_t* xc_tile_base;
  const uint16_t* xc_t_pos;
  double* xc;
};

struct SweepArgs {
  const BundleDesc* bundles;
  const uint2* in_arcs;
  const uint2* out_arcs;
  const uint32_t* in_off;
  const uint32_t* out_off;
  const uint32_t* level_off;
  const uint32_t* pair_start;
  const uint32_t* pair_final;
  const uint32_t* pair_id;
  const double* pair_logw;
  const double* logw;
  double* post;
  double* scalars;
  double* pair_logprob;
  double* val_g;
  double* val2_g;
  uint32_t first_bundle;
};

struct WaveArgs {
  const WaveDesc* descs;
  const uint2* fwd;
  const uint32_t* bwd;
  const uint32_t* level_off;
  const uint32_t* frow;
  const uint32_t* brow;
  const double* wcache;
  const double* logw = nullptr;
  const uint32_t* bwd_arc = nullptr;
  uint32_t n_arcs = 0;
  double* xc = nullptr;
  const uint32_t* xc_idx = nullptr;
  double* post;
  double* pair_logprob;
  double* spill;
  uint32_t first;
  uint32_t max_states, max_width;
};

struct ReduceArgs {
  const uint64_t* arc_off;
  const uint64_t* slot_pos;
  const uint64_t* hot_chunks;
  const double* post;
  double* counts;
  uint64_t n_arcs, n_hot_chunks;
};

struct TransArgs {
  const TransBucket* buckets;
  const uint64_t* tile_base;
  const uint16_t* b_arc;
  const uint16_t* b_rank;
  const uint32_t* b_src;
  const uint16_t* t_pos;
  const uint32_t* t_src;
  const uint16_t* a_off;
  double* x;
  double* xc;
  const double* logw;
  double* wcache;
  const double* post;
  double* counts;
  uint64_t n_wcache, n_post;
  uint32_t n_buckets, n_tiles;
  uint32_t n_wtiles;
  const uint32_t* tr_off;
  const uint16_t* tr_rel;
  const uint32_t* tr_src;
  const uint32_t* br_off;
  const uint16_t* br_rel;
  const uint32_t* br_src;
  uint32_t use_runs;
  uint32_t scatter;
  uint32_t tile;
  uint32_t bucket;
  uint32_t tile_first, tile_count;
  uint32_t bucket_first, bucket_count;
  uint32_t slack_bytes;
  const uint32_t* zero_list = nullptr;
  uint32_t n_zero = 0;
};

#define TRANS_RUN_CAP 4096
#define TRANS_RUN_LDS (TRANS_RUN_CAP * 4 + 4096)
#define MSTEP_BIG_GROUP 48
#define MSTEP_PARTIALS 2048
#define MSTEP_MAX_RANGES 17
#define MSTEP_WIDE_SLOTS 512
#define MSTEP_WIDE_SHARDS 32
#define MSTEP_WIDE_TICKETS (16 * (MSTEP_WIDE_SHARDS + 1))
struct MstepArgs {
  double* logw;
  const double* lw_src;
  double* old_logw;
  const double* counts;
  const double* prior;
  const uint32_t* group;
  const uint32_t* norm_of;
  const double* add_count;
  const uint64_t* group_off;
  const uint64_t* norm_perm;
  const uint64_t* big_groups;
  uint64_t n_groups, n_big;
  double* gscale;
  unsigned long long* max_partial;
  unsigned long long* max_change_bits;
  int all_grouped;
  uint32_t window_span;
  double* glocked;
  const uint32_t* tie_of;
  double* tie_tab;
  uint64_t n_ties;
  uint64_t n;
  uint32_t block_first;
  uint32_t n_ranges;
  uint32_t range_first[MSTEP_MAX_RANGES];
  uint32_t range_cum[MSTEP_MAX_RANGES + 1];
  int save_old;
  const uint32_t* mask32;
  const uint32_t* lockmask32;
  const unsigned long long* mask64;
  const unsigned long long* lockmask64;
  const uint16_t* code16;
  const double* dig_alpha;
  const double* tie_alpha;
  unsigned long long* box = nullptr;
  unsigned long long box_seq = 0;
  unsigned long long* ticket = nullptr;
};

hipError_t launch_lane_sweep(const LaneArgs& A, const LatticeSet::LaneClass& lc, hipStream_t stream, bool fused = false);
hipError_t launch_sweep(const SweepArgs& A, const LatticeSet::LaunchClass& lc, hipStream_t stream);
hipError_t launch_wave_sweep(const WaveArgs& A, const LatticeSet::WaveClass& wc, hipStream_t stream);
hipError_t launch_trans_w_bucket(const TransArgs& T, hipStream_t stream);
hipError_t launch_trans_w_bucket_range(const TransArgs& T, uint32_t first, uint32_t count, hipStream_t stream);
hipError_t launch_trans_c_bucket_range(const TransArgs& T, uint32_t first, uint32_t count, hipStream_t stream);
hipError_t launch_tile_sweep(const TransArgs& T, const LaneArgs& A, const uint32_t* tile_group, uint32_t tile_first, uint32_t tile_count,
                             hipStream_t stream);
hipError_t launch_pack_tile_records(const LaneGroup* groups, uint32_t n_groups, const uint32_t* lane_nstates, const uint32_t* fwdx,
                                    const uint32_t* bwd, uint32_t* out, uint32_t* chain, const uint32_t* tile_group, uint32_t n_tiles,
                                    uint32_t* tile_chain, hipStream_t stream);
hipError_t launch_zero_list(double* p, const uint32_t* idx, uint32_t n, hipStream_t stream);
hipError_t launch_gather_idx(double* small, const double* src, const uint32_t* idx, uint32_t n, hipStream_t stream);
hipError_t launch_scatter_idx(double* dst, const double* small, const uint32_t* idx, uint32_t n, hipStream_t stream);
hipError_t launch_mstep_window_range(const MstepArgs& M, int use_counts, uint32_t block_first, uint32_t n_blocks, hipStream_t s);
hipError_t launch_mstep_max_final(const MstepArgs& M, hipStream_t s);
hipError_t launch_trans_w_tiles(const TransArgs& T, uint32_t tile_first, uint32_t tile_count, hipStream_t stream);
hipError_t launch_trans_c_tiles(const TransArgs& T, uint32_t tile_first, uint32_t tile_count, hipStream_t stream);
hipError_t launch_trans_c_bucket(const TransArgs& T, const uint32_t* split_arcs, uint32_t n_split, hipStream_t stream);
hipError_t launch_scalars(const double* pair_logprob, const double* pair_w, uint64_t n_pairs, double* partial,
                          double* scalars, hipStream_t s);
hipError_t launch_count_reduce(const ReduceArgs& R, hipStream_t stream);
hipError_t launch_fill(double* p, double v, uint64_t n, hipStream_t s);
hipError_t launch_add(double* dst, const double* src, uint64_t n, hipStream_t s);
hipError_t launch_mstep(const MstepArgs& M, int use_counts, hipStream_t s);
bool mstep_wide_can(const MstepArgs& M, int use_counts);
hipError_t launch_mstep_wide(const MstepArgs& M, int use_counts, uint32_t grid_cap, hipStream_t s);
hipError_t launch_overrelax(double* logw, const double* old_logw, double* em_logw, const uint32_t* group, double rate,
                            uint64_t n, hipStream_t s);
hipError_t launch_max_change(const double* logw, const double* old_logw, const uint32_t* group,
                             unsigned long long* bits, uint64_t n, hipStream_t s);
hipError_t launch_chain_update(double* arc_logw, const uint32_t* arc_chain, const uint64_t* chain_off,
                               const uint64_t* chain_param, const double* param_logw, uint64_t n_arcs, hipStream_t s);
hipError_t launch_chain_scatter(double* param_counts, const double* arc_counts, double arc_prior, const double* arc_prior_w,
                                const uint32_t* arc_chain, const uint64_t* chain_off, const uint64_t* chain_param,
                                const uint32_t* param_group, uint64_t n_arcs, hipStream_t s);
hipError_t launch_counts_to_logw(double* logw, const double* counts, const double* prior, const uint32_t* group, uint64_t n,
                                 hipStream_t s);

}
```

### carmel_amd/csrc/lattice_gpu.hip

```cpp
#include <hip/hip_runtime.h>
#include <hipcub/hipcub.hpp>
#include <algorithm>
#include <chrono>
#include <functional>
#include <cmath>
#include <cstring>
#include <limits>
#include <vector>
#include "engine.hpp"
#include "options.hpp"

namespace {

struct GCaps {
  uint32_t cx, ce, ck, ch, threads;
};
const GCaps G_SMALL = {256, 448, 256, 512, 131072};
const GCaps G_LARGE = {1024, 2560, 1536, 2048, 65536};

enum { PF_HAS = 1, PF_FALLBACK = 2 };

struct GArgs {
  const uint64_t* idx_off;
  const uint64_t* idx_key;
// ... 1076 lines not shown
  HIPCHK(rec_bwd.alloc(np * GK));
  HIPCHK(rec_arc.alloc(np * GK));
  GArgs G;
  G.idx_off = d_idx_off.p;
  G.idx_key = d_idx_key.p;
  G.idx_arc = d_idx_arc.p;
  G.arc_dst = d_dst.p;
  G.final_state = w.final_state;
  G.in_off = d_in_off.p;
  G.out_off = d_out_off.p;
  G.in_sym = d_in.p;
  G.out_sym = d_out.p;
  G.n_pairs = np;
  G.lane_states = opt.lane_states;
  G.cx = GX;
  G.ce = GE;
  G.ck = GK;
  G.ch = GH;
  G.span_min = opt.lane_window ? opt.lane_window_min : 0xffffffffu;
  G.pp_span = pp_span.p;
  G.pp_L = pp_L.p;
  G.scratch = scratch.p;
  G.scratch_stride = stride;
  G.pp_E = pp_E.p;
  G.pp_S = pp_S.p;
  G.pp_flags = pp_flags.p;
  G.pp_xs = pp_xs.p;
  G.pp_xa = pp_xa.p;
  G.rec_fwd = rec_fwd.p;
  G.rec_bwd = rec_bwd.p;
  G.rec_arc = rec_arc.p;
  lap("uploads");
  hipLaunchKernelGGL(explore_kernel, dim3(n_threads / 256), dim3(256), 0, s, G);
  HIPCHK(hipGetLastError());
  DevBuf<unsigned long long> d_stats;
  HIPCHK(d_stats.alloc(8));
  HIPCHK(hipMemsetAsync(d_stats.p, 0, 64, s));
  hipLaunchKernelGGL(pair_stats_kernel, dim3(1024), dim3(256), 0, s, pp_E.p, pp_S.p, pp_flags.p, pp_xs.p, pp_xa.p, np, opt.lane_window_min, d_stats.p);
  unsigned long long hs[8];
  HIPCHK(hipMemcpyAsync(hs, d_stats.p, 64, hipMemcpyDeviceToHost, s));
  HIPCHK(hipStreamSynchronize(s));
  lap("explore + prune + records");
  if (hs[1]) return CARMEL_HIP_OK;
  const uint64_t n_kept = hs[0], n_items = hs[5];
  if (!n_kept || n_items >= (1ull << 32) || np >= (1ull << 32)) return CARMEL_HIP_OK;
  const uint32_t use_window = (opt.lane_window && hs[6] * 10 >= hs[5]) ? 1u : 0u;
  unsigned long long hc[4] = {0, 0, 0, 0};
  {
    ClassArgs CA;
    CA.E = pp_E.p;
    CA.S = pp_S.p;
    CA.span = pp_span.p;
    CA.L = pp_L.p;
    CA.flags = pp_flags.p;
    CA.n = np;
    CA.use_window = use_window;
    CA.lane_window = opt.lane_window;
    CA.lane_states = opt.lane_states;
    CA.wave_min_width = opt.wave_lane_min_width;
    CA.wave_lane_arcs = opt.wave ? opt.wave_lane_arcs : 0xffffffffu;
    HIPCHK(hipMemsetAsync(d_stats.p, 0, 64, s));
    hipLaunchKernelGGL(classify_kernel, dim3(1024), dim3(256), 0, s, CA, pp_win.p, d_stats.p);
    HIPCHK(hipMemcpyAsync(hc, d_stats.p, 32, hipMemcpyDeviceToHost, s));
    HIPCHK(hipStreamSynchronize(s));
  }
  const uint64_t n_plain = hc[0], n_win = hc[1];
  if (hc[2]) return CARMEL_HIP_OK;
  if (opt.wave && hc[3] && n_plain + n_win < opt.wave_lane_threshold) return CARMEL_HIP_OK;
  DevBuf<unsigned long long> key, key_sorted;
  DevBuf<char> tmp;
  HIPCHK(key.alloc(np));
  HIPCHK(key_sorted.alloc(np));
  hipLaunchKernelGGL(pair_key_kernel, dim3((unsigned)((np + 255) / 256)), dim3(256), 0, s, pp_E.p, pp_S.p, pp_flags.p, pp_win.p, np, key.p);
  HIPCHK(sort_keys(tmp, key.p, key_sorted.p, np, 64, s));
  const size_t ng_plain = (size_t)((n_plain + 63) / 64), ng = ng_plain + (size_t)((n_win + 63) / 64);
  SlotMap SM;
  SM.n_plain = n_plain;
  SM.n_win = n_win;
  SM.ng_plain = (uint32_t)ng_plain;
  DevBuf<uint32_t> g_maxlen, g_maxstates, g_items, g_window;
  HIPCHK(g_maxlen.alloc(ng));
  HIPCHK(g_maxstates.alloc(ng));
  HIPCHK(g_items.alloc(ng));
  HIPCHK(g_window.alloc(ng));
  hipLaunchKernelGGL(group_dims_kernel, dim3((unsigned)ng), dim3(64), 0, s, key_sorted.p, pp_E.p, pp_S.p, pp_win.p, SM, g_maxlen.p,
                     g_maxstates.p, g_items.p, g_window.p);
  std::vector<uint32_t> h_maxlen(ng), h_maxstates(ng), h_items(ng), h_window(ng);
  HIPCHK(hipMemcpyAsync(h_maxlen.data(), g_maxlen.p, ng * 4, hipMemcpyDeviceToHost, s));
  HIPCHK(hipMemcpyAsync(h_maxstates.data(), g_maxstates.p, ng * 4, hipMemcpyDeviceToHost, s));
  HIPCHK(hipMemcpyAsync(h_items.data(), g_items.p, ng * 4, hipMemcpyDeviceToHost, s));
  HIPCHK(hipMemcpyAsync(h_window.data(), g_window.p, ng * 4, hipMemcpyDeviceToHost, s));
  HIPCHK(hipStreamSynchronize(s));
  LatticeSet& L = t->lat;
  L = LatticeSet();
  L.lane_groups.resize(ng);
  std::vector<unsigned long long> h_item_off(ng);
  uint64_t spill_rows = 0;
  {
    unsigned long long acc = 0;
    for (size_t g = 0; g < ng; ++g) {
      LaneGroup& Gd = L.lane_groups[g];
      std::memset(&Gd, 0, sizeof Gd);
      Gd.n_lanes = (uint32_t)(g < ng_plain ? std::min<uint64_t>(64, n_plain - g * 64) : std::min<uint64_t>(64, n_win - (g - ng_plain) * 64));
      Gd.pair_base = (uint32_t)(g * 64);
      Gd.maxlen = h_maxlen[g];
      const uint32_t win = g < ng_plain ? 0u : h_window[g];
      Gd.max_states = win ? win : h_maxstates[g];
      Gd.window = win;
      if (win) {
        if (spill_rows + h_maxstates[g] > 0xffffffffull) return CARMEL_HIP_OK;
        Gd.spill_row = (uint32_t)spill_rows;
        spill_rows += h_maxstates[g];
      }
      h_item_off[g] = acc;
      acc += h_items[g];
    }
  }
  L.lane_spill_rows = spill_rows;
  const uint64_t n_rec = assign_lane_classes(L, opt, true);
  if (n_rec >= (1ull << 32)) return CARMEL_HIP_OK;
  lap("pair sort + lane groups");
  HIPCHK(t->lane_groups.upload(L.lane_groups, s));
  if (L.tile_sweep)
    HIPCHK(t->tile_group.upload(L.tile_group, s));
  else
    t->tile_group.release();
  DevBuf<unsigned long long> d_item_off, items, items_sorted;
  HIPCHK(d_item_off.upload(h_item_off, s));
  HIPCHK(t->lane_fwdx.alloc(n_rec));
  t->lane_fwd.release();
  HIPCHK(t->lane_bwd.alloc(n_rec));
  HIPCHK(hipMemsetAsync(t->lane_fwdx.p, 0, n_rec * 4, s));
  HIPCHK(hipMemsetAsync(t->lane_bwd.p, 0, n_rec * 4, s));
  HIPCHK(t->lane_pair.alloc(ng * 64));
  HIPCHK(t->lane_nstates.alloc(ng * 64));
  HIPCHK(t->lane_logw.alloc(ng * 64));
  HIPCHK(items.alloc(n_items));
  HIPCHK(items_sorted.alloc(n_items));
  hipLaunchKernelGGL(interleave_kernel, dim3((unsigned)ng), dim3(64), 0, s, t->lane_groups.p, key_sorted.p, pp_E.p, pp_S.p, rec_fwd.p,
                     rec_bwd.p, rec_arc.p, d_pw.p, SM, GK, d_item_off.p, t->lane_fwdx.p, t->lane_bwd.p, t->lane_pair.p,
                     t->lane_nstates.p, t->lane_logw.p, items.p);
  if (spill_rows)
    HIPCHK(t->lane_spill.alloc(spill_rows * 64));
  else
    t->lane_spill.release();
  HIPCHK(hipGetLastError());
  if (L.tile_sweep) {
    HIPCHK(t->lane_rec2.alloc(n_rec));
    HIPCHK(t->lane_chain.alloc(ng));
    HIPCHK(t->tile_chain.alloc(t->tile_group.n - 1));
    HIPCHK(hipMemsetAsync(t->lane_rec2.p, 0, n_rec * 4, s));
    HIPCHK(launch_pack_tile_records(t->lane_groups.p, (uint32_t)t->lane_groups.n, t->lane_nstates.p, t->lane_fwdx.p, t->lane_bwd.p, t->lane_rec2.p, t->lane_chain.p,
                                    t->tile_group.p, (uint32_t)(t->tile_group.n - 1), t->tile_chain.p, s));
    if (lib_opt("timing")) {
      std::vector<uint32_t> ch(t->lane_chain.n);
      HIPCHK(hipMemcpyAsync(ch.data(), t->lane_chain.p, ch.size() * 4, hipMemcpyDeviceToHost, s));
      HIPCHK(hipStreamSynchronize(s));
      size_t n1 = 0;
      for (uint32_t c : ch) n1 += c & 1u;
      fprintf(stderr, "timing: tile sweep: %zu tiles, %zu groups, %zu of them single paths\n", L.tile_group.size() - 1, ch.size(), n1);
    }
  } else {
    t->lane_rec2.release();
    t->lane_chain.release();
    t->tile_chain.release();
  }
  lap("record streams");
  {
    int rc = gpu_tables_from_items(t, tmp, items, items_sorted, n_items, n_items,  n_rec, lap);
    if (rc) return rc;
  }
  const uint64_t n_post = n_rec;
  t->use_transpose = true;
  t->lane_records = n_rec;
  t->wave_descs.release();
  t->wave_fwd.release();
  t->wave_bwd.release();
  t->wave_bwd_arc.release();
  t->wave_level_off.release();
  t->wave_frow.release();
  t->wave_brow.release();
  t->wave_spill.release();
  t->wave_slot_base = n_rec;
  t->wave_records = 0;
  if (L.lane_fused)
    t->post.release();
  else
    HIPCHK(t->post.alloc(n_post));
  HIPCHK(t->wcache.alloc(n_rec));
  t->bundles.release();
  t->in_arcs.release();
  t->out_arcs.release();
  t->in_off.release();
  t->out_off.release();
  t->level_off.release();
  t->pair_start.release();
  t->pair_final.release();
  t->pair_id.release();
  t->pair_logw.release();
  t->alpha_g.release();
  t->beta_g.release();
  std::vector<uint8_t> flags(np);
  HIPCHK(hipMemcpyAsync(flags.data(), pp_flags.p, np, hipMemcpyDeviceToHost, s));
  HIPCHK(hipStreamSynchronize(s));
  L.has_deriv.resize(np);
  std::vector<double> pw(np);
  for (uint64_t p = 0; p < np; ++p) {
    L.has_deriv[p] = (flags[p] & PF_HAS) ? 1 : 0;
    pw[p] = L.has_deriv[p] ? (c.weight.empty() ? 1.0 : c.weight[p]) : -1.0;
  }
  if (has_derivation) std::memcpy(has_derivation, L.has_deriv.data(), np);
  HIPCHK(t->pair_w.upload(pw, s));
  HIPCHK(t->scalar_partial.alloc(3 * 256));
  HIPCHK(t->pair_logprob.alloc(np));
  HIPCHK(launch_fill(t->pair_logprob.p, -std::numeric_limits<double>::infinity(), np, s));
  uint32_t last_xs = 0;
  HIPCHK(hipMemcpyAsync(&last_xs, pp_xs.p + (np - 1), 4, hipMemcpyDeviceToHost, s));
  uint64_t last_kept = np;
  while (last_kept > 0 && !L.has_deriv[last_kept - 1]) --last_kept;
  uint16_t lastS = 0, lastE = 0;
  if (last_kept) {
    HIPCHK(hipMemcpyAsync(&lastS, pp_S.p + (last_kept - 1), 2, hipMemcpyDeviceToHost, s));
    HIPCHK(hipMemcpyAsync(&lastE, pp_E.p + (last_kept - 1), 2, hipMemcpyDeviceToHost, s));
  }
  HIPCHK(hipStreamSynchronize(s));
  L.n_kept = n_kept;
  L.explored_states = hs[2];
  L.explored_arcs = hs[3];
  L.total_states = hs[4];
  L.total_arcs = hs[5];
  L.lane_states = hs[4];
  L.lane_arcs = hs[5];
  L.n_post = n_post;
  L.last_pre_states = last_xs;
  L.last_post_states = lastS;
  L.last_post_arcs = lastE;
  {
    uint64_t ml = 0;
    for (auto& g : L.lane_groups) ml = std::max<uint64_t>(ml, g.max_states);
    L.max_levels = ml;
  }
  t->device_bytes = t->lane_groups.bytes() + t->lane_fwdx.bytes() + t->lane_bwd.bytes() + t->lane_pair.bytes() + t->lane_nstates.bytes() +
                    t->lane_logw.bytes() + t->post.bytes() + t->wcache.bytes() + t->arc_off.bytes() + t->slot_pos.bytes() +
                    t->t_b_arc.bytes() + t->t_b_rank.bytes() + t->t_t_pos.bytes() + t->t_b_src.bytes() + t->t_t_src.bytes() +
                    t->t_x.bytes() + t->t_xc.bytes() + t->pair_logprob.bytes() + t->lane_spill.bytes();
  t->have_lattices = true;
  ++t->lattice_epoch;
  if (stats) {
    std::memset(stats, 0, sizeof *stats);
    stats->n_pairs = np;
    stats->n_pairs_kept = n_kept;
    stats->explored_states = L.explored_states;
    stats->explored_arcs = L.explored_arcs;
    stats->kept_states = L.total_states;
    stats->kept_arcs = L.total_arcs;
    stats->n_bundles = L.lane_groups.size();
    stats->max_levels = L.max_levels;
    stats->device_bytes = t->device_bytes;
    stats->build_seconds = std::chrono::duration<double>(std::chrono::steady_clock::now() - t0).count();
    stats->last_pair_explored_states = L.last_pre_states;
    stats->last_pair_kept_states = L.last_post_states;
    stats->last_pair_kept_arcs = L.last_post_arcs;
    stats->n_windowed_pairs = n_win;
    stats->n_windowed_pairs = 0;
    for (auto& g : L.lane_groups)
      if (g.window) stats->n_windowed_pairs += g.n_lanes;
  }
  lap("finish");
  done = true;
  return CARMEL_HIP_OK;
}
```

### carmel_amd/csrc/options.cpp

```cpp
#include "options.hpp"
#include <cstdlib>
#include <cstring>
#include <mutex>
#include <string>
#include "../../include/carmel_hip.h"

namespace carmel_hip {
namespace {
const char* const kKeys[] = {
    "timing",
    "lane_states", "tile_sweep", "lane_fused", "transpose", "lane_chunks", "lane_window", "lane_window_min", "wave_ring", "wave_min_width",
    "gpu_build", "wave_gather", "wave_xc", "tile_gather", "device_tables", "trans_scatter", "trans_runs", "lane_fused_kernel",
    "tile_sweep_kernel", "mailbox", "poison", "lane_trace", "exchange_sparse", "mstep_wide",
    "dense", "unrolled", "unrolled_ragged",
    "gibbs_chains", "gibbs_own_cap", "gibbs_workgroup", "gibbs_clk", "gibbs_reg", "gibbs_lane", "forest_sweep", "forest_ldswalk", "forest_multi",
    "forest_nohash", "forest_trace", "forest_exact_host", "forest_exact_clk", "forest_logdomain", "forest_gcol", "forest_gather",
    "decode_lds", "decode_chunk_bytes"};
constexpr int kN = (int)(sizeof kKeys / sizeof kKeys[0]);
const char* volatile g_val[kN];
std::mutex g_mu;
int find(const char* key) {
  for (int i = 0; i < kN; ++i)
    if (!std::strcmp(kKeys[i], key)) return i;
  return -1;
}
}
const char* lib_opt(const char* key) {
  const int i = find(key);
  return i < 0 ? nullptr : g_val[i];
}
bool lib_opt_off(const char* key) {
  const char* v = lib_opt(key);
  return v && std::atoi(v) == 0;
}
}

extern "C" {
int carmel_hip_set_option(const char* key, const char* value) {
  using namespace carmel_hip;
  if (!key) return CARMEL_HIP_ERR_ARG;
  const int i = find(key);
  if (i < 0) return CARMEL_HIP_ERR_ARG;
  std::lock_guard<std::mutex> lk(g_mu);
  if (!value)
    g_val[i] = nullptr;
  else {
    char* c = (char*)std::malloc(std::strlen(value) + 1);
    if (!c) return CARMEL_HIP_ERR_HIP;
    std::strcpy(c, value);
    g_val[i] = c;
  }
  return CARMEL_HIP_OK;
}
const char* carmel_hip_get_option(const char* key) { return key ? carmel_hip::lib_opt(key) : nullptr; }
int carmel_hip_option_count(void) { return carmel_hip::kN; }
const char* carmel_hip_option_name(int i) { return i >= 0 && i < carmel_hip::kN ? carmel_hip::kKeys[i] : nullptr; }
}
```

### carmel_amd/csrc/tile_sweep.hip

```cpp
#include "kernels.hpp"
#include "sweep_math.hpp"
#include <algorithm>

namespace carmel_hip {

#define TS_SRC(x) ((x) & 0xffu)
#define TS_POS(x) (((x) >> 8) & 63u)
#define TS_FV 0x4000u
#define TS_FL 0x8000u
#define TS_DST(x) (((x) >> 16) & 0xffu)
#define TS_BV 0x1000000u
#define TS_BL 0x2000000u
#define TS_FCHAIN 0x4000000u
#define TS_FEASY 0x8000000u
#define TS_BCHAIN 0x10000000u
#define TS_BEASY 0x20000000u
__global__ void pack_tile_records_kernel(const LaneGroup* __restrict__ groups, uint32_t n_groups, const uint32_t* __restrict__ lane_nstates,
                                         const uint32_t* __restrict__ fwdx, const uint32_t* __restrict__ bwd, uint32_t* __restrict__ out,
                                         uint32_t* __restrict__ chain) {
  const uint32_t gi = blockIdx.x * (blockDim.x >> 6) + (threadIdx.x >> 6), lane = threadIdx.x & 63;
  if (gi >= n_groups) return;
  const LaneGroup g = groups[gi];
  const uint32_t S = lane < g.n_lanes ? lane_nstates[g.pair_base + lane] : 0u;
  uint32_t d = 1, s = S >= 2 ? S - 2 : 0u;
// ... 209 lines not shown
                                                   double* rows) {
  constexpr int U = (int)LANE_CHUNK;
  const bool active = (uint32_t)lane < g.n_lanes;
  const uint32_t S = active ? L.S : 0u;
  const uint32_t len = S ? S - 1 : 0u;
  const uint32_t maxlen = g.maxlen;
  const uint32_t off = maxlen - len;
  for (uint32_t k = 0; k < max_pad; ++k)
    if (k < off) rows[k * 64] = 0.0;
  col[0] = 0.0;
  double prev = 0.0;
  {
    const double* wr = rows + (size_t)(maxlen - 1) * 64;
    double* cw = col + 64;
    double wa[U], wb[U];
#pragma unroll
    for (int u = 0; u < U; ++u) wa[u] = wr[-u * 64];
    for (uint32_t kb = 0; kb < maxlen; kb += 2 * U) {
      const bool two = kb + U < maxlen;
      if (two) {
#pragma unroll
        for (int u = 0; u < U; ++u) wb[u] = wr[-(U + u) * 64];
      }
#pragma unroll
      for (int u = 0; u < U; ++u) {
        prev += wa[u];
        cw[u * 64] = prev;
      }
      if (kb + 2 * U < maxlen) {
#pragma unroll
        for (int u = 0; u < U; ++u) wa[u] = wr[-(2 * U + u) * 64];
      }
      if (two) {
#pragma unroll
        for (int u = 0; u < U; ++u) {
          prev += wb[u];
          cw[(U + u) * 64] = prev;
        }
      }
      wr -= 2 * U * 64;
      cw += 2 * U * 64;
    }
  }
  const double lp = prev;
  double next = (!active || lp == NEG_INF) ? NEG_INF : L.lwt - lp;
  {
    double* wr = rows;
    double* ca = col + (size_t)(maxlen - 1) * 64;
    double wa[U], aa[U], wb[U], ab[U];
#pragma unroll
    for (int u = 0; u < U; ++u) {
      wa[u] = wr[u * 64];
      aa[u] = ca[-u * 64];
    }
    for (uint32_t kb = 0; kb < maxlen; kb += 2 * U) {
      const bool two = kb + U < maxlen;
      if (two) {
#pragma unroll
        for (int u = 0; u < U; ++u) {
          wb[u] = wr[(U + u) * 64];
          ab[u] = ca[-(U + u) * 64];
        }
      }
#pragma unroll
      for (int u = 0; u < U; ++u) {
        next = wa[u] + next;
        ca[-u * 64] = next;
        wr[u * 64] = aa[u] + next;
      }
      if (kb + 2 * U < maxlen) {
#pragma unroll
        for (int u = 0; u < U; ++u) {
          wa[u] = wr[(2 * U + u) * 64];
          aa[u] = ca[-(2 * U + u) * 64];
        }
      }
      if (two) {
#pragma unroll
        for (int u = 0; u < U; ++u) {
          next = wb[u] + next;
          ca[-(U + u) * 64] = next;
          wr[(U + u) * 64] = ab[u] + next;
        }
      }
      wr += 2 * U * 64;
      ca -= 2 * U * 64;
    }
  }
  return lp;
}
#define TILE_SWEEP_THREADS 512
#define TILE_SWEEP_MOVERS 256
typedef uint32_t ts_u32x4 __attribute__((ext_vector_type(4)));
struct TileIn {
  double v[TILE_SWEEP_TILE / TILE_SWEEP_MOVERS];
  uint16_t pos[TILE_SWEEP_TILE / TILE_SWEEP_MOVERS];
};
template <bool SCAT>
__device__ __forceinline__ void tile_request(const TransArgs& T, const LaneArgs& A, uint32_t tile, uint64_t i0, uint32_t ni, uint32_t m,
                                             TileIn& in) {
  constexpr int NM = TILE_SWEEP_MOVERS, KT = (int)(TILE_SWEEP_TILE / NM);
  const uint16_t* __restrict__ tp = T.t_pos + i0 + m;
#pragma unroll
  for (int k = 0; k < KT; ++k) in.pos[k] = tp[k * NM];
  if (SCAT) {
    const double* __restrict__ xp = T.x + i0 + m;
#pragma unroll
    for (int k = 0; k < KT; ++k) in.v[k] = xp[k * NM];
  } else {
    const uint32_t last = ni ? ni - 1 : 0u;
    const uint32_t* __restrict__ sp = T.t_src + (ni ? i0 : 0);
    uint32_t src[KT];
#pragma unroll
    for (int k = 0; k < KT; ++k) src[k] = sp[min(m + k * NM, last)];
#pragma unroll
    for (int k = 0; k < KT; ++k) in.v[k] = T.x[src[k]];
  }
}
__device__ __forceinline__ void tile_exp_in_place(double* lds) {
  constexpr int K = (int)(TILE_SWEEP_TILE / TILE_SWEEP_THREADS);
#pragma unroll
  for (int k0 = 0; k0 < K; k0 += 4) {
    double v[4];
#pragma unroll
    for (int k = 0; k < 4; ++k) v[k] = lds[threadIdx.x + (k0 + k) * TILE_SWEEP_THREADS];
#pragma unroll
    for (int k = 0; k < 4; ++k) lds[threadIdx.x + (k0 + k) * TILE_SWEEP_THREADS] = K_EXP(v[k]);
    __builtin_amdgcn_sched_barrier(0);
  }
}
__device__ __forceinline__ uint32_t ts_zero() {
  uint32_t z = 0;
  asm volatile("" : "+v"(z));
  return z;
}
__device__ __forceinline__ uint32_t ts_sc(uint32_t v) { return __builtin_amdgcn_readfirstlane(v); }
__device__ __forceinline__ uint64_t ts_sc(uint64_t v) { return ((uint64_t)ts_sc((uint32_t)(v >> 32)) << 32) | ts_sc((uint32_t)v); }
__device__ __forceinline__ LaneGroup ts_uniform(const LaneGroup& v) {
  LaneGroup g;
  g.stream_base = ts_sc(v.stream_base);
  g.maxlen = ts_sc(v.maxlen);
  g.n_lanes = ts_sc(v.n_lanes);
  g.pair_base = ts_sc(v.pair_base);
  g.max_states = ts_sc(v.max_states);
  g.window = 0;
  g.spill_row = ts_sc(v.spill_row);
  return g;
}
struct TileWalk {
  uint32_t tile, ni, g0, g1, chain;
  uint64_t i0, i1;
  bool ok;
};
__device__ __forceinline__ TileWalk tile_walk_at(const TransArgs& T, const LaneArgs& A, const uint32_t* __restrict__ tile_group, uint32_t vidx,
                                                 bool ok, uint32_t z) {
  TileWalk w;
  const uint32_t tloc = xcd_chunked(vidx, T.tile_count);
  w.ok = ok && tloc < T.tile_count && vidx / 8 < (T.tile_count + 7) / 8;
  w.tile = T.tile_first + (w.ok ? tloc : 0u);
  w.i0 = T.tile_base[w.tile + z];
  w.i1 = T.tile_base[w.tile + 1 + z];
  w.g0 = tile_group[w.tile + z];
  w.g1 = tile_group[w.tile + 1 + z];
  w.chain = A.tile_chain[w.tile + z];
  w.ni = 0;
  return w;
}
__device__ __forceinline__ TileWalk ts_uniform(const TileWalk& v) {
  TileWalk w;
  w.tile = v.tile;
  w.ok = v.ok;
  w.i0 = ts_sc(v.i0);
  w.i1 = ts_sc(v.i1);
  w.ni = (uint32_t)(w.i1 - w.i0);
  w.g0 = ts_sc(v.g0);
  w.g1 = ts_sc(v.g1);
  w.chain = ts_sc(v.chain);
  return w;
}
template <bool SCAT>
__global__ __launch_bounds__(TILE_SWEEP_THREADS) void tile_sweep_kernel(TransArgs T, LaneArgs A, const uint32_t* __restrict__ tile_group) {
  extern __shared__ __attribute__((aligned(16))) double lds[];
  constexpr int NM = TILE_SWEEP_MOVERS, KT = (int)(TILE_SWEEP_TILE / NM), NW = (TILE_SWEEP_THREADS - NM) / 64;
  uint32_t* const recs = (uint32_t*)(lds + TILE_SWEEP_TILE);
  double* const alpha = lds + TILE_SWEEP_TILE + TILE_SWEEP_TILE / 2;
  const int lane = threadIdx.x & 63;
  const uint32_t wv = __builtin_amdgcn_readfirstlane(threadIdx.x >> 6);
  uint32_t vidx = blockIdx.x;
  const uint32_t z = ts_zero();
  for (uint32_t i = blockIdx.x * TILE_SWEEP_THREADS + threadIdx.x; i < T.n_zero; i += gridDim.x * TILE_SWEEP_THREADS) T.counts[T.zero_list[i]] = 0.0;
  TileWalk cur = tile_walk_at(T, A, tile_group, vidx, true, z);
  if (!cur.ok) return;
  cur = ts_uniform(cur);
  TileWalk nxt = ts_uniform(tile_walk_at(T, A, tile_group, vidx + gridDim.x, true, z));
  TileWalk nn_raw = tile_walk_at(T, A, tile_group, vidx + 2 * gridDim.x, nxt.ok, z);
  if (wv >= (uint32_t)NW) {
    const uint32_t m = threadIdx.x - (uint32_t)(TILE_SWEEP_THREADS - NM);
    TileIn in;
    tile_request<SCAT>(T, A, cur.tile, cur.i0, cur.ni, m, in);
    const uint32_t mw = wv - (uint32_t)NW;
    LaneGroup gm_raw;
    TileLane lm;
    uint32_t cm_raw;
    {
      const uint32_t gk = cur.g0 + NW + mw < cur.g1 ? cur.g0 + NW + mw : cur.g0;
      gm_raw = A.groups[gk + z];
      lm = tile_lane(A, gk, lane);
      cm_raw = A.chain[gk + z];
    }
    for (;;) {
      uint32_t pos2[KT / 2];
#pragma unroll
      for (int k = 0; k < KT; ++k) {
        if (k & 1)
          pos2[k / 2] |= (uint32_t)in.pos[k] << 16;
        else
          pos2[k / 2] = in.pos[k];
        if (m + k * NM < cur.ni) lds[in.pos[k]] = in.v[k];
      }
      __syncthreads();
      if (nxt.ok) tile_request<SCAT>(T, A, nxt.tile, nxt.i0, nxt.ni, m, in);
      {
        const LaneGroup gm = ts_uniform(gm_raw);
        const TileLane lm_cur = lm;
        const uint32_t cm = ts_sc(cm_raw);
        const bool mine = cur.g0 + NW + mw < cur.g1 && (cm & 1u);
        const uint32_t gk = nxt.g0 + NW + mw < nxt.g1 ? nxt.g0 + NW + mw : nxt.g0;
        gm_raw = A.groups[gk + z];
        lm = tile_lane(A, gk, lane);
        cm_raw = A.chain[gk + z];
        if (mine) {
          const uint32_t off = (uint32_t)(gm.stream_base - (uint64_t)cur.tile * TILE_SWEEP_TILE) + lane;
          const double lp = tile_chain_sweep(gm, lm_cur, cm >> 8, lane, alpha + (size_t)gm.spill_row * 64 + lane, lds + off);
          if ((uint32_t)lane < gm.n_lanes) A.pair_logprob[lm_cur.pair] = lp;
        }
      }
      uint32_t dst[KT];
      __builtin_amdgcn_sched_barrier(0);
      if (SCAT) {
        const uint32_t* __restrict__ sp = T.t_src + cur.i0 + m;
#pragma unroll
        for (int k = 0; k < KT; ++k) dst[k] = sp[k * NM];
      }
      __syncthreads();
      tile_exp_in_place(lds);
      __syncthreads();
#pragma unroll
      for (int k = 0; k < KT; ++k) {
        const uint32_t i = m + k * NM;
        const uint32_t q = (k & 1) ? pos2[k / 2] >> 16 : pos2[k / 2] & 0xffffu;
        if (i < cur.ni) T.xc[SCAT ? (uint64_t)dst[k] : cur.i0 + i] = lds[q];
      }
      if (!nxt.ok) break;
      __syncthreads();
      vidx += gridDim.x;
      cur = nxt;
      nxt = ts_uniform(nn_raw);
      nn_raw = tile_walk_at(T, A, tile_group, vidx + 2 * gridDim.x, nxt.ok, z);
    }
  } else {
    constexpr int KR = (int)(TILE_SWEEP_TILE / 4 / (TILE_SWEEP_THREADS - NM));
    LaneGroup g;
    TileLane L;
    uint32_t chain;
    {
      const uint32_t gk = cur.g0 + wv < cur.g1 ? cur.g0 + wv : cur.g0;
      g = ts_uniform(A.groups[gk + z]);
      L = tile_lane(A, gk, lane);
      chain = ts_sc(A.chain[gk + z]);
      if (!cur.chain) {
        ts_u32x4 rr[KR];
#pragma unroll
        for (int k = 0; k < KR; ++k)
          rr[k] = *(const ts_u32x4*)(A.rec2 + (uint64_t)cur.tile * TILE_SWEEP_TILE + (threadIdx.x + k * (TILE_SWEEP_THREADS - NM)) * 4);
#pragma unroll
        for (int k = 0; k < KR; ++k) *(ts_u32x4*)(recs + (threadIdx.x + k * (TILE_SWEEP_THREADS - NM)) * 4) = rr[k];
      }
    }
    for (;;) {
      unsigned long long t0 = 0, t1 = 0, t2 = 0;
      if (A.trace) t0 = __builtin_readcyclecounter();
      const uint64_t p0 = (uint64_t)cur.tile * TILE_SWEEP_TILE;
      const uint32_t gk_n = nxt.g0 + wv < nxt.g1 ? nxt.g0 + wv : nxt.g0;
      const LaneGroup g_n = A.groups[gk_n + z];
      const TileLane L_n = tile_lane(A, gk_n, lane);
      const uint32_t chain_n = A.chain[gk_n + z];
      __syncthreads();
      if (A.trace) t1 = __builtin_readcyclecounter();
      for (uint32_t gi = cur.g0 + wv; gi < cur.g1; gi += NW) {
        const uint32_t gk = gi + NW < cur.g1 ? gi + NW : gi;
        const LaneGroup g_next = A.groups[gk + z];
        const TileLane L_next = tile_lane(A, gk, lane);
        const uint32_t chain_next = A.chain[gk + z];
        const uint32_t off = (uint32_t)(g.stream_base - p0) + lane;
        const bool movers = gi == cur.g0 + NW + wv && (chain & 1u);
        double lp = 0.0;
        if (!movers) {
          if (chain & 1u)
            lp = tile_chain_sweep(g, L, chain >> 8, lane, alpha + (size_t)g.spill_row * 64 + lane, lds + off);
          else
            lp = tile_group_sweep(g, L, lane, alpha + (size_t)g.spill_row * 64 + lane, lds + off, recs + off);
        }
        const bool active = !movers && (uint32_t)lane < g.n_lanes;
        const uint32_t pair = L.pair;
        g = ts_uniform(g_next);
        chain = ts_sc(chain_next);
        L = L_next;
        if (active) A.pair_logprob[pair] = lp;
      }
      if (A.trace && lane == 0) A.trace[(size_t)cur.tile * 16 + 8 + wv] = __builtin_readcyclecounter() - t1;
      const bool recs_n = nxt.ok && !nxt.chain;
      ts_u32x4 rr[KR];
      if (recs_n) {
#pragma unroll
        for (int k = 0; k < KR; ++k)
          rr[k] = *(const ts_u32x4*)(A.rec2 + (uint64_t)nxt.tile * TILE_SWEEP_TILE + (threadIdx.x + k * (TILE_SWEEP_THREADS - NM)) * 4);
      }
      __syncthreads();
      if (A.trace) t2 = __builtin_readcyclecounter();
      tile_exp_in_place(lds);
      __syncthreads();
      if (recs_n) {
#pragma unroll
        for (int k = 0; k < KR; ++k) *(ts_u32x4*)(recs + (threadIdx.x + k * (TILE_SWEEP_THREADS - NM)) * 4) = rr[k];
      }
      if (A.trace && threadIdx.x == 0) {
        unsigned long long* o = A.trace + (size_t)cur.tile * 16;
        o[0] = t0;
        o[1] = t1 - t0;
        o[2] = t2 - t1;
        o[4] = ((unsigned long long)(cur.g1 - cur.g0) << 32) | cur.ni;
        o[5] = ((unsigned long long)__builtin_amdgcn_s_getreg((4 << 0) | (0 << 6) | (31 << 11)) << 32) | g.maxlen;
      }
      if (!nxt.ok) break;
      __syncthreads();
      if (A.trace && threadIdx.x == 0) A.trace[(size_t)cur.tile * 16 + 3] = __builtin_readcyclecounter() - t2;
      vidx += gridDim.x;
      cur = nxt;
      nxt = ts_uniform(nn_raw);
      nn_raw = tile_walk_at(T, A, tile_group, vidx + 2 * gridDim.x, nxt.ok, z);
      g = ts_uniform(g_n);
      L = L_n;
      chain = ts_sc(chain_n);
    }
  }
}
#define TRANS_SET_LDS(K, BYTES) (void)hipFuncSetAttribute((const void*)K, hipFuncAttributeMaxDynamicSharedMemorySize, BYTES)
hipError_t launch_tile_sweep(const TransArgs& T0, const LaneArgs& A, const uint32_t* tile_group, uint32_t tile_first, uint32_t tile_count,
                             hipStream_t stream) {
  if (!T0.n_buckets || !tile_count) return hipSuccess;
  if (T0.tile != TILE_SWEEP_TILE || !A.pre_weights || !A.rec2 || !A.chain || !A.tile_chain) return hipErrorInvalidValue;
  if (T0.slack_bytes < TILE_SWEEP_TILE * sizeof(double)) return hipErrorInvalidValue;
  int dev = 0;
  if (hipGetDevice(&dev) != hipSuccess || dev < 0 || dev >= 64) return hipErrorInvalidDevice;
  static int dev_cus[64] = {0};
  const int lds = (int)TILE_SWEEP_LDS;
  if (!dev_cus[dev]) {
    if (hipFuncSetAttribute((const void*)tile_sweep_kernel<false>, hipFuncAttributeMaxDynamicSharedMemorySize, lds) != hipSuccess ||
        hipFuncSetAttribute((const void*)tile_sweep_kernel<true>, hipFuncAttributeMaxDynamicSharedMemorySize, lds) != hipSuccess)
      return hipErrorInvalidValue;
    hipDeviceProp_t prop;
    if (hipGetDeviceProperties(&prop, dev) != hipSuccess) return hipErrorInvalidDevice;
    __atomic_store_n(&dev_cus[dev], prop.multiProcessorCount > 8 ? prop.multiProcessorCount / 8 * 8 : 8, __ATOMIC_RELEASE);
  }
  const int n_cu = __atomic_load_n(&dev_cus[dev], __ATOMIC_ACQUIRE);
  TransArgs T = T0;
  T.tile_first = tile_first;
  T.tile_count = tile_count;
  const dim3 g8(std::min<uint32_t>((uint32_t)n_cu, (tile_count + 7) / 8 * 8));
  if ((T.scatter & 3u) == 3u && T.use_runs)
    hipLaunchKernelGGL((tile_sweep_kernel<true>), g8, dim3(TILE_SWEEP_THREADS), lds, stream, T, A, tile_group);
  else if (!(T.scatter & 3u))
    hipLaunchKernelGGL((tile_sweep_kernel<false>), g8, dim3(TILE_SWEEP_THREADS), lds, stream, T, A, tile_group);
  else
    return hipErrorInvalidValue;
  return hipGetLastError();
}
hipError_t launch_pack_tile_records(const LaneGroup* groups, uint32_t n_groups, const uint32_t* lane_nstates, const uint32_t* fwdx,
                                    const uint32_t* bwd, uint32_t* out, uint32_t* chain, const uint32_t* tile_group, uint32_t n_tiles,
                                    uint32_t* tile_chain, hipStream_t stream) {
  if (n_groups)
    hipLaunchKernelGGL(pack_tile_records_kernel, dim3((n_groups + 3) / 4), dim3(256), 0, stream, groups, n_groups, lane_nstates, fwdx, bwd, out,
                       chain);
  if (n_tiles) hipLaunchKernelGGL(tile_chain_kernel, dim3((n_tiles + 255) / 256), dim3(256), 0, stream, tile_group, chain, n_tiles, tile_chain);
  return hipGetLastError();
}
}
```

### carmel_amd/trainer.py

```python
import ctypes as C
import math

import numpy as np

from . import _capi
from ._capi import EstimateResult, LatticeStats, check, lib, ptr
from .model import NORM_CONDITIONAL


class TrainOpts(object):

    def __init__(self, max_iter=500, converge_arc_delta=1e-4, converge_ppx_ratio=.999,
                 learning_rate_growth_factor=1.0):
        self.max_iter = max_iter
        self.converge_arc_delta = converge_arc_delta
        self.converge_ppx_ratio = converge_ppx_ratio
        self.learning_rate_growth_factor = learning_rate_growth_factor


class HipComm(object):

    @staticmethod
    def unique_id():
        buf = (C.c_char * 128)()
        check(lib.carmel_hip_comm_unique_id(buf), "carmel_hip_comm_unique_id")
        return bytes(buf.raw)

    def __init__(self, device, rank, world, id_bytes):
        assert len(id_bytes) == 128
        h = C.c_void_p()
        check(lib.carmel_hip_comm_create(C.byref(h), device, rank, world, C.c_char_p(id_bytes)), "carmel_hip_comm_create")
        self.h, self.rank, self.world = h, rank, world

    @classmethod
    def custom(cls, plugin_path, session, device, rank, world):
        plug = C.CDLL(plugin_path)
        tr = (C.c_void_p * 6)()
        plug.carmel_hip_transport_open.argtypes = [C.c_char_p, C.c_int, C.c_int, C.c_int, C.c_void_p]
        rc = plug.carmel_hip_transport_open(session.encode(), rank, world, device, C.cast(tr, C.c_void_p))
        if rc != 0:
            raise RuntimeError("carmel_hip_transport_open(%s) failed: %d" % (plugin_path, rc))
        self = cls.__new__(cls)
        h = C.c_void_p()
        check(lib.carmel_hip_comm_create_custom(C.byref(h), device, rank, world, C.cast(tr, C.c_void_p)), "carmel_hip_comm_create_custom")
        self.h, self.rank, self.world, self._plug = h, rank, world, plug
        if hasattr(plug, "carmel_hip_transport_sendrecv"):
            check(lib.carmel_hip_comm_set_sendrecv(h, C.cast(plug.carmel_hip_transport_sendrecv, C.c_void_p)), "carmel_hip_comm_set_sendrecv")
        return self

    @property
    def transport(self):
        return lib.carmel_hip_comm_transport_name(self.h).decode()

    def allreduce_host(self, values, op_max=False):
        v = np.ascontiguousarray(values, dtype=np.float64).copy()
        check(lib.carmel_hip_comm_allreduce_host(self.h, ptr(v), len(v), 1 if op_max else 0), "carmel_hip_comm_allreduce_host")
        return v

    def selftest(self, n=0):
        check(lib.carmel_hip_comm_selftest(self.h, n), "carmel_hip_comm_selftest")

    def abort(self):
        if self.h:
            lib.carmel_hip_comm_abort(self.h)
            self.h = None

    def close(self):
        if self.h:
            lib.carmel_hip_comm_destroy(self.h)
            self.h = None

    def __del__(self):
        try:
            self.close()
        except Exception:
            pass


class HipForwardBackward(object):
    def __init__(self, wfst, corpus, norm_group=NORM_CONDITIONAL, add_count=0.0, smooth_floor=0.0,
                 weight_is_prior_count=False, device=0, prune=True, host_threads=0, cascade=None,
                 normalize_first=True):
        self.wfst, self.corpus = wfst, corpus
        h = C.c_void_p()
        check(lib.carmel_hip_create(C.byref(h), device, wfst.n_states, wfst.final, wfst.n_arcs, ptr(wfst.src),
                                    ptr(wfst.dst), ptr(wfst.isym), ptr(wfst.osym), ptr(wfst.logw), ptr(wfst.group)),
              "carmel_hip_create")
        self.h = h
        self.cascade = cascade
        if cascade is not None:
            c = cascade
            check(lib.carmel_hip_set_cascade(
                h, len(c["param_logw"]), ptr(c["param_logw"]), ptr(c["param_group"]), ptr(c["param_member"]),
                ptr(c["param_src"]), ptr(c["param_in"]), len(c["member_norm"]), ptr(c["member_norm"]),
                ptr(c["member_add_count"]), len(c["chain_off"]) - 1, ptr(c["chain_off"]), ptr(c["chain_param"])),
                "carmel_hip_set_cascade")
            self.n_params = len(c["param_logw"])
        else:
            check(lib.carmel_hip_set_norm(h, norm_group, add_count), "carmel_hip_set_norm")
            self.n_params = wfst.n_arcs
        if normalize_first:
            check(lib.carmel_hip_normalize(h), "carmel_hip_normalize")
        if cascade is None or smooth_floor:
            check(lib.carmel_hip_set_prior(h, smooth_floor, 1 if weight_is_prior_count else 0), "carmel_hip_set_prior")
        check(lib.carmel_hip_set_corpus(h, corpus.n_pairs, ptr(corpus.in_off), ptr(corpus.in_sym),
                                        ptr(corpus.out_off), ptr(corpus.out_sym), ptr(corpus.weight)),
              "carmel_hip_set_corpus")
        self.has_deriv = np.zeros(corpus.n_pairs, dtype=np.uint8)
        self.lattice_stats = LatticeStats()
        check(lib.carmel_hip_build_lattices(h, 1 if prune else 0, host_threads, ptr(self.has_deriv),
                                            C.byref(self.lattice_stats)), "carmel_hip_build_lattices")
        self.stats = corpus.stats(self.has_deriv.astype(bool))
        self.last = None

    def rebuild_lattices(self, prune=True, host_threads=0):
        check(lib.carmel_hip_build_lattices(self.h, 1 if prune else 0, host_threads, ptr(self.has_deriv),
                                            C.byref(self.lattice_stats)), "carmel_hip_build_lattices")

    def close(self):
        if self.h:
            lib.carmel_hip_destroy(self.h)
            self.h = None

    def __del__(self):
        try:
            self.close()
        except Exception:
            pass

    def estimate(self, per_pair=False):
        res = EstimateResult()
        pp = np.empty(self.corpus.n_pairs) if per_pair else None
        check(lib.carmel_hip_estimate(self.h, C.byref(res), ptr(pp)), "carmel_hip_estimate")
        self.last = res
        self.pair_logprob = pp
        return res.sum_logprob, res.sum_weighted_logprob

    def estimate_async(self):
        check(lib.carmel_hip_estimate_async(self.h), "carmel_hip_estimate_async")

    def synchronize(self):
        check(lib.carmel_hip_synchronize(self.h), "carmel_hip_synchronize")

    def allreduce_counts(self, comm):
        check(lib.carmel_hip_allreduce_counts(self.h, comm.h), "carmel_hip_allreduce_counts")

    def layout_description(self):
        ls, lay = self.lattice_stats, lib.carmel_hip_lattice_layout(self.h)
        if lay == 1:
            return "unrolled over string positions (never stored)"
        if lay == 2:
            return "unrolled, rank-1 dense form (never stored)"
        tiles, fused = lib.carmel_hip_lattice_tile_sweep(self.h), lib.carmel_hip_lattice_fused_lanes(self.h)
        src = self.weight_source
        return "explicit: %d lattices, %d of them windowed; %d lane groups + bundles; %.2f GB in HBM%s%s%s%s" % (
            ls.n_pairs_kept, ls.n_windowed_pairs, ls.n_bundles, ls.device_bytes / 1e9,
            "; laid out for the tile sweep (%d tiles)" % tiles if tiles else "",
            "; fused lanes (%d tiles)" % fused if fused else "",
            "; weights from the WFST's table (%s)" % " and ".join(
                n for b, n in ((1, "tile passes"), (2, "wave sweeps")) if src & b) if src & 3 else "",
            "; wave posteriors straight to the count pass" if src & 4 else "")

    @property
    def weight_source(self):
        return lib.carmel_hip_lattice_weight_source(self.h)

    @property
    def tile_sweep_tiles(self):
        return lib.carmel_hip_lattice_tile_sweep(self.h)

    @property
    def fused_lane_tiles(self):
        return lib.carmel_hip_lattice_fused_lanes(self.h)

    EXCHANGE_FORMS = {"auto": 0, "allreduce": 1, "collectives": 2, "direct": 3}

    def exchange_plan(self, comm, n_chunks=0, force_allreduce=False, form="auto"):
        f = 1 if force_allreduce else self.EXCHANGE_FORMS[form]
        check(lib.carmel_hip_exchange_plan(self.h, comm.h, n_chunks, f), "carmel_hip_exchange_plan")
        self._comm = comm
        return self.exchange_info()

    def exchange_info(self):
        sh, k = C.c_int(0), C.c_uint32(0)
        rs, ag, ar = C.c_uint64(0), C.c_uint64(0), C.c_uint64(0)
        check(lib.carmel_hip_exchange_info(self.h, C.byref(sh), C.byref(k), C.byref(rs), C.byref(ag), C.byref(ar)),
              "carmel_hip_exchange_info")
        return dict(sharded=bool(sh.value), form=("allreduce", "collectives", "direct")[sh.value], n_chunks=k.value, bytes_reduce_scatter=rs.value, bytes_all_gather=ag.value,
                    bytes_all_reduce=ar.value)

    def exchange_measure(self, reps=5):
        ms = C.c_double(0)
        check(lib.carmel_hip_exchange_measure(self.h, reps, C.byref(ms)), "carmel_hip_exchange_measure")
        return ms.value

    def exchange_clear(self):
        check(lib.carmel_hip_exchange_clear(self.h), "carmel_hip_exchange_clear")
        self._comm = None

    def set_matrix_fb(self, on=True):
        check(lib.carmel_hip_set_matrix_fb(self.h, int(on)), "carmel_hip_set_matrix_fb")

    def set_layout_policy(self, allow_unrolled):
        check(lib.carmel_hip_set_layout_policy(self.h, int(allow_unrolled)), "carmel_hip_set_layout_policy")

    def last_kernel_ms(self):
        ms = C.c_double(0)
        check(lib.carmel_hip_last_sweep_ms(self.h, C.byref(ms)), "carmel_hip_last_sweep_ms")
        return ms.value

    def read_scalars(self):
        res = EstimateResult()
        check(lib.carmel_hip_read_scalars(self.h, C.byref(res)), "carmel_hip_read_scalars")
        return res.sum_logprob, res.sum_weighted_logprob, res.n_pairs

    def use_external_counts(self, dev_ptr):
        check(lib.carmel_hip_use_external_counts(self.h, C.c_void_p(dev_ptr)), "carmel_hip_use_external_counts")

    def counts(self):
        out = np.empty(self.wfst.n_arcs)
        check(lib.carmel_hip_get_counts(self.h, ptr(out)), "carmel_hip_get_counts")
        return out

    def maximize(self, delta_scale=1.0):
        mc = C.c_double(0)
        check(lib.carmel_hip_maximize(self.h, delta_scale, C.byref(mc)), "carmel_hip_maximize")
        return mc.value

    def keep_em_weights(self):
        check(lib.carmel_hip_keep_em_weights(self.h), "carmel_hip_keep_em_weights")

    def weights(self):
        out = np.empty(self.n_params)
        check(lib.carmel_hip_get_weights(self.h, ptr(out)), "carmel_hip_get_weights")
        return out

    def arc_weights(self):
        out = np.empty(self.wfst.n_arcs)
        check(lib.carmel_hip_get_arc_weights(self.h, ptr(out)), "carmel_hip_get_arc_weights")
        return out

    def set_weights(self, logw):
        logw = np.ascontiguousarray(logw, dtype=np.float64)
        assert len(logw) == self.n_params
        check(lib.carmel_hip_set_weights(self.h, ptr(logw)), "carmel_hip_set_weights")

    def save_counts(self):
        check(lib.carmel_hip_save_counts(self.h), "carmel_hip_save_counts")

    def save_best(self):
        check(lib.carmel_hip_save_best(self.h), "carmel_hip_save_best")

    def load_best(self):
        check(lib.carmel_hip_load_best(self.h), "carmel_hip_load_best")


def _rel_ppx_ratio_ln(new_ppx_ln, old_ppx_ln):
    if new_ppx_ln == 0:
        return float("nan")
    return (new_ppx_ln - old_ppx_ln) / abs(new_ppx_ln)


def train(fb, opts=None, log=None):
    opts = opts or TrainOpts()
    using_cascade = fb.cascade is not None
    st = fb.stats
    W = st["total_weight"]
    n_sym = max(st["n_input"], st["n_output"])
    best = float("inf")
    have_good = False
    last_change = 10.0
    last_ppx = float("inf")
    learning_rate = 1.0
    growth = 1.0 if using_cascade else opts.learning_rate_growth_factor
    trace = []
    it = 0
    last_was_reset = False
    while True:
        first_time = it == 0
        it += 1
        cascade_counts = using_cascade and not first_time
        if cascade_counts:
            fb.save_counts()
        if opts.max_iter is not None and it > opts.max_iter and have_good:
            break
        lp, wlp = fb.estimate()
        tol = 4.45e-16 * max(st["n_pairs"], 1)
        lp, wlp = (0.0 if abs(lp) <= tol else lp), (0.0 if abs(wlp) <= tol else wlp)
        new_ppx = -wlp / W
        rec = dict(iter=it, log2_prob=lp / math.log(2), log2_ppx_symbol=(-lp / n_sym) / math.log(2) if n_sym else 0.0,
                   log2_ppx_example=(-lp / st["n_pairs"]) / math.log(2), n_symbol=n_sym, n_example=st["n_pairs"],
                   new_best=False, rel_ppx_ratio_ln=float("nan"), last_change=last_change, rate=learning_rate)
        if new_ppx < best and (not using_cascade or cascade_counts):
            rec["new_best"] = True
            best = new_ppx
            have_good = True
            fb.save_best()
        if first_time:
            ratio_ln = -float("inf")
        else:
            ratio_ln = _rel_ppx_ratio_ln(new_ppx, last_ppx)
            rec["rel_ppx_ratio_ln"] = ratio_ln
        trace.append(rec)
        if log:
            log(rec)
        if not last_was_reset:
            if ratio_ln >= math.log(opts.converge_ppx_ratio):
                if learning_rate > 1:
                    learning_rate = 1.0
                    fb.keep_em_weights()
                    last_was_reset = True
                    continue
                if have_good:
                    break
            elif learning_rate < 20:
                learning_rate *= growth
        else:
            last_was_reset = False
        last_change = fb.maximize(learning_rate)
        if last_change <= opts.converge_arc_delta and have_good:
            break
        last_ppx = new_ppx
# ... 80 lines not shown
```

### include/carmel_hip.h

```cpp
#ifndef CARMEL_HIP_H
#define CARMEL_HIP_H
#include <stdint.h>
#ifdef __cplusplus
extern "C" {
#endif

#define CARMEL_HIP_OK 0
#define CARMEL_HIP_ERR_ARG -1
#define CARMEL_HIP_ERR_HIP -2
#define CARMEL_HIP_ERR_STATE -3
#define CARMEL_HIP_ERR_NO_DERIV -4
#define CARMEL_HIP_ERR_UNSUPPORTED -5

#define CARMEL_HIP_NO_GROUP 0xFFFFFFFFu
#define CARMEL_HIP_LOCKED_GROUP 0u

#define CARMEL_HIP_NORM_CONDITIONAL 0
#define CARMEL_HIP_NORM_JOINT 1
#define CARMEL_HIP_NORM_NONE 2

typedef struct carmel_hip_trainer carmel_hip_trainer;

const char* carmel_hip_last_error(void);
int carmel_hip_set_option(const char* key, const char* value);
const char* carmel_hip_get_option(const char* key);
int carmel_hip_option_count(void);
const char* carmel_hip_option_name(int i);
int carmel_hip_device_count(void);

int carmel_hip_create(carmel_hip_trainer** out, int device, uint32_t n_states, uint32_t final_state, uint64_t n_arcs,
                      const uint32_t* src, const uint32_t* dst, const uint32_t* in_sym, const uint32_t* out_sym,
                      const double* logw, const uint32_t* group);
int carmel_hip_destroy(carmel_hip_trainer* t);

int carmel_hip_set_corpus(carmel_hip_trainer* t, uint64_t n_pairs, const uint64_t* in_off, const uint32_t* in_sym,
                          const uint64_t* out_off, const uint32_t* out_sym, const double* pair_weight);

typedef struct carmel_hip_lattice_stats {
  uint64_t n_pairs;
  uint64_t n_pairs_kept;
  uint64_t explored_states;
  uint64_t explored_arcs;
  uint64_t kept_states;
  uint64_t kept_arcs;
  uint64_t n_cyclic_pairs;
  uint64_t n_bundles;
  uint64_t max_levels;
  uint64_t device_bytes;
  double build_seconds;
  uint64_t last_pair_explored_states, last_pair_kept_states, last_pair_kept_arcs;
  uint64_t n_windowed_pairs;
} carmel_hip_lattice_stats;

int carmel_hip_build_lattices(carmel_hip_trainer* t, int prune, int host_threads, uint8_t* has_derivation,
                              carmel_hip_lattice_stats* stats);

int carmel_hip_debug_lattice_fingerprint(carmel_hip_trainer* t, uint64_t* out16);
int carmel_hip_lattice_tile_sweep(carmel_hip_trainer* t);
int carmel_hip_lattice_fused_lanes(carmel_hip_trainer* t);
int carmel_hip_lattice_weight_source(carmel_hip_trainer* t);
int carmel_hip_lattice_layout(carmel_hip_trainer* t);

int carmel_hip_set_norm(carmel_hip_trainer* t, int norm_group_by, double add_count);

int carmel_hip_set_prior(carmel_hip_trainer* t, double smooth_floor, int weight_is_prior_count);

int carmel_hip_set_cascade(carmel_hip_trainer* t, uint64_t n_params, const double* param_logw,
                           const uint32_t* param_group, const uint32_t* param_member, const uint32_t* param_src,
                           const uint32_t* param_in, uint32_t n_members, const int* member_norm,
                           const double* member_add_count, uint64_t n_chains, const uint64_t* chain_off,
                           const uint64_t* chain_param);

int carmel_hip_normalize(carmel_hip_trainer* t);

int carmel_hip_set_weights(carmel_hip_trainer* t, const double* logw);
int carmel_hip_get_weights(carmel_hip_trainer* t, double* logw);
int carmel_hip_get_arc_weights(carmel_hip_trainer* t, double* logw);

typedef struct carmel_hip_estimate_result {
  double sum_logprob;
  double sum_weighted_logprob;
  uint64_t n_pairs;
  double kernel_ms;
} carmel_hip_estimate_result;

int carmel_hip_estimate(carmel_hip_trainer* t, carmel_hip_estimate_result* res, double* per_pair_logprob);
int carmel_hip_estimate_async(carmel_hip_trainer* t);
int carmel_hip_estimate_finish(carmel_hip_trainer* t, carmel_hip_estimate_result* res, double* per_pair_logprob);

void* carmel_hip_counts_dev(carmel_hip_trainer* t);
uint64_t carmel_hip_counts_len(carmel_hip_trainer* t);
void* carmel_hip_stream(carmel_hip_trainer* t);
int carmel_hip_use_external_counts(carmel_hip_trainer* t, void* dev_ptr);
int carmel_hip_synchronize(carmel_hip_trainer* t);
int carmel_hip_last_sweep_ms(carmel_hip_trainer* t, double* ms);
int carmel_hip_read_scalars(carmel_hip_trainer* t, carmel_hip_estimate_result* res);
int carmel_hip_get_counts(carmel_hip_trainer* t, double* counts );
int carmel_hip_set_counts(carmel_hip_trainer* t, const double* counts );
int carmel_hip_accumulate_counts(carmel_hip_trainer* t, int op);

int carmel_hip_maximize(carmel_hip_trainer* t, double delta_scale, double* max_change);

int carmel_hip_fractional_counts(carmel_hip_trainer* t);

int carmel_hip_set_digamma(carmel_hip_trainer* t, uint32_t n_members, const double* alpha, const uint8_t* enabled);

int carmel_hip_random_restart(carmel_hip_trainer* t, uint64_t seed, uint32_t restart);
int carmel_hip_keep_em_weights(carmel_hip_trainer* t);
int carmel_hip_save_counts(carmel_hip_trainer* t);
int carmel_hip_save_best(carmel_hip_trainer* t);
int carmel_hip_load_best(carmel_hip_trainer* t);

typedef struct carmel_hip_comm carmel_hip_comm;
int carmel_hip_comm_unique_id(void* id128);
int carmel_hip_comm_create(carmel_hip_comm** out, int device, int rank, int world, const void* id128);
int carmel_hip_comm_destroy(carmel_hip_comm* c);
int carmel_hip_comm_abort(carmel_hip_comm* c);
int carmel_hip_comm_rank(carmel_hip_comm* c);
int carmel_hip_comm_world(carmel_hip_comm* c);
const char* carmel_hip_comm_transport_name(carmel_hip_comm* c);
int carmel_hip_allreduce_counts(carmel_hip_trainer* t, carmel_hip_comm* c);
int carmel_hip_comm_allreduce_host(carmel_hip_comm* c, double* v, uint32_t n, int op_max);

typedef struct carmel_hip_transport {
  void* ctx;
  int (*allreduce)(void* ctx, double* dev_buf, uint64_t n, int op, void* stream);
  int (*reduce_scatter)(void* ctx, double* dev_buf, uint64_t count, void* stream);
  int (*all_gather)(void* ctx, double* dev_buf, uint64_t count, void* stream);
  void (*destroy)(void* ctx);
  const char* name;
} carmel_hip_transport;
int carmel_hip_comm_create_custom(carmel_hip_comm** out, int device, int rank, int world, const carmel_hip_transport* tr);
typedef struct carmel_hip_p2p {
  int32_t peer;
  int32_t send;
  double* dev_buf;
  uint64_t n;
} carmel_hip_p2p;
typedef int (*carmel_hip_sendrecv_fn)(void* ctx, const carmel_hip_p2p* ops, uint32_t n_ops, void* stream);
int carmel_hip_comm_set_sendrecv(carmel_hip_comm* c, carmel_hip_sendrecv_fn fn);
int carmel_hip_comm_selftest(carmel_hip_comm* c, uint32_t n);

int carmel_hip_exchange_plan(carmel_hip_trainer* t, carmel_hip_comm* c, uint32_t n_chunks, int form);
int carmel_hip_exchange_info(carmel_hip_trainer* t, int* sharded, uint32_t* n_chunks, uint64_t* bytes_reduce_scatter,
                             uint64_t* bytes_all_gather, uint64_t* bytes_all_reduce);
int carmel_hip_exchange_measure(carmel_hip_trainer* t, uint32_t reps, double* ms_per_exchange);
int carmel_hip_exchange_clear(carmel_hip_trainer* t);
int carmel_hip_set_layout_policy(carmel_hip_trainer* t, int allow_unrolled);
int carmel_hip_set_matrix_fb(carmel_hip_trainer* t, int on);

typedef struct carmel_hip_gibbs carmel_hip_gibbs;
typedef struct carmel_hip_gibbs_opts {
  uint32_t iter;
  uint32_t burnin;
  uint64_t seed;
  int mode;
  int uniform_p0, dirichlet_p0, final_counts, exclude_prior;
  double min_prior;
  double high_temp, low_temp;
  int expectation;
  uint32_t restarts;
  int argmax_final, argmax_sum;
  int include_self;
  int random_start;
} carmel_hip_gibbs_opts;
int carmel_hip_gibbs_create(carmel_hip_gibbs** out, carmel_hip_trainer* t, const carmel_hip_gibbs_opts* opts);
int carmel_hip_gibbs_destroy(carmel_hip_gibbs* g);
uint32_t carmel_hip_gibbs_n_blocks(carmel_hip_gibbs* g);
int carmel_hip_gibbs_lattice_stats(carmel_hip_gibbs* g, carmel_hip_lattice_stats* stats);
uint32_t carmel_hip_gibbs_max_sample(carmel_hip_gibbs* g);
int carmel_hip_gibbs_run(carmel_hip_gibbs* g, double* iter_logprob, double* iter_cheap_logprob);
int carmel_hip_gibbs_run_ex(carmel_hip_gibbs* g, double* iter_logprob, double* iter_cheap_logprob, double* iter_after_logprob);
int carmel_hip_gibbs_set_run_share(carmel_hip_gibbs* g, uint32_t first, uint32_t stride);
int carmel_hip_gibbs_best_stats(carmel_hip_gibbs* g, double* out3, int* ran_any);

int carmel_hip_gibbs_set_prior_inference(carmel_hip_gibbs* g, double stddev, int global, int local, int restart_fresh,
                                         uint32_t start, uint32_t end, const int* member_priorgroup,
                                         const uint32_t* member_n_states, uint32_t n_members);
int carmel_hip_gibbs_prior_trace(carmel_hip_gibbs* g, double* out6, uint32_t n_sweeps, double* cumulative, uint32_t n_cumulative);
uint32_t carmel_hip_gibbs_n_prior_scales(carmel_hip_gibbs* g);

typedef void (*carmel_hip_gibbs_observer_fn)(void* ctx, uint32_t run, uint32_t iter, double time);
int carmel_hip_gibbs_set_observer(carmel_hip_gibbs* g, uint32_t every, carmel_hip_gibbs_observer_fn fn, void* ctx);
int carmel_hip_gibbs_current_probs(carmel_hip_gibbs* g, double* prob);
int carmel_hip_gibbs_get_state(carmel_hip_gibbs* g, double* x, double* sum, double* tmax, double* prior, double* last_touch);
int carmel_hip_gibbs_final_counts(carmel_hip_gibbs* g, double* x);
int carmel_hip_gibbs_get_sample(carmel_hip_gibbs* g, uint32_t block, uint32_t* ids, uint32_t* n);
int carmel_hip_gibbs_set_init_weights(carmel_hip_gibbs* g, const double* arc_logw);
uint32_t carmel_hip_gibbs_best_run(carmel_hip_gibbs* g);
double carmel_hip_gibbs_uniform(uint64_t seed, uint32_t iter, uint32_t block, uint32_t step);
double carmel_hip_gibbs_power(double high_temp, double low_temp, uint32_t iter, uint32_t sweep);

typedef struct carmel_hip_forests carmel_hip_forests;
int carmel_hip_forests_create(carmel_hip_forests** out, int device, uint64_t n_forests, const uint64_t* node_off,
                              const uint32_t* label, const int32_t* ref, const uint32_t* next, uint32_t n_rules,
                              const double* rule_logw, uint64_t n_groups, const uint64_t* group_off,
                              const uint32_t* group_rule);
int carmel_hip_forests_destroy(carmel_hip_forests* f);
int carmel_hip_forests_estimate(carmel_hip_forests* f, double prior_count, double* avg_logprob, uint64_t* n_zero,
                                double* per_forest_logprob);
int carmel_hip_forests_get_counts(carmel_hip_forests* f, double prior_count, double* counts );
int carmel_hip_forests_maximize(carmel_hip_forests* f, double prior_count, double add_k, int zero_zerocounts,
                                double* max_delta);
int carmel_hip_forests_get_weights(carmel_hip_forests* f, double* rule_logw);
int carmel_hip_forests_set_weights(carmel_hip_forests* f, const double* rule_logw);
int carmel_hip_forests_gibbs(carmel_hip_forests* f, const carmel_hip_gibbs_opts* opts, double alpha,
                             double* iter_logprob, double* iter_cheap_logprob);
uint32_t carmel_hip_forests_best_run(carmel_hip_forests* f);
int carmel_hip_forests_final_counts(carmel_hip_forests* f, double* x );
int carmel_hip_forests_set_prior_inference(carmel_hip_forests* F, double stddev, int global, int local, uint32_t start,
                                           uint32_t end);
// ... 67 lines not shown
```

Baseline: 53.11 billion arc-updates/s.

## Balance tile-sweep work across workgroups with a cost-model static schedule

```diff
diff --git a/carmel_amd/_capi.py b/carmel_amd/_capi.py
--- a/carmel_amd/_capi.py
+++ b/carmel_amd/_capi.py
@@ -26,7 +26,7 @@
     "carmel_hip_forests_max_sample", "carmel_hip_forests_viterbi", "carmel_hip_forests_get_viterbi",
     "carmel_hip_compose", "carmel_hip_composition_states", "carmel_hip_composition_arcs", "carmel_hip_composition_seconds",
     "carmel_hip_composition_export", "carmel_hip_composition_free",
-    "carmel_hip_debug_lattice_fingerprint", "carmel_hip_lattice_layout", "carmel_hip_lattice_tile_sweep", "carmel_hip_lattice_fused_lanes", "carmel_hip_lattice_weight_source", "carmel_hip_accumulate_counts",
+    "carmel_hip_debug_lattice_fingerprint", "carmel_hip_lattice_layout", "carmel_hip_lattice_tile_sweep", "carmel_hip_tile_schedule", "carmel_hip_lattice_tile_schedule", "carmel_hip_lattice_fused_lanes", "carmel_hip_lattice_weight_source", "carmel_hip_accumulate_counts",
     "carmel_hip_comm_unique_id", "carmel_hip_comm_create", "carmel_hip_comm_destroy", "carmel_hip_comm_rank",
     "carmel_hip_comm_world", "carmel_hip_allreduce_counts", "carmel_hip_comm_allreduce_host",
     "carmel_hip_comm_abort", "carmel_hip_comm_transport_name", "carmel_hip_comm_create_custom", "carmel_hip_comm_set_sendrecv", "carmel_hip_comm_selftest", "carmel_hip_exchange_plan",
@@ -183,6 +183,9 @@
     lib.carmel_hip_gibbs_best_stats.argtypes = [vp, vp, vp]
     lib.carmel_hip_lattice_layout.argtypes = [vp]
     lib.carmel_hip_lattice_tile_sweep.argtypes = [vp]
+    u32p = C.POINTER(C.c_uint32)
+    lib.carmel_hip_tile_schedule.argtypes = [u32p, u32p, u32p, C.c_uint32, C.c_uint32, u32p, u32p, C.POINTER(C.c_double)]
+    lib.carmel_hip_lattice_tile_schedule.argtypes = [vp, u32p, u32p, u32p, u32p]
     lib.carmel_hip_lattice_fused_lanes.argtypes = [vp]
     lib.carmel_hip_lattice_weight_source.argtypes = [vp]
     lib.carmel_hip_accumulate_counts.argtypes = [vp, C.c_int]
diff --git a/carmel_amd/csrc/engine.cpp b/carmel_amd/csrc/engine.cpp
--- a/carmel_amd/csrc/engine.cpp
+++ b/carmel_amd/csrc/engine.cpp
@@ -11,6 +11,7 @@
 #include <vector>
 #include "engine.hpp"
 #include "options.hpp"
+#include "tile_schedule.hpp"
 #include "host/refhash.hpp"
 #include "rng.hpp"
 #include "unrolled_args.hpp"
@@ -334,6 +335,7 @@
     HIPCHK(hipMemsetAsync(t->lane_rec2.p, 0, t->lane_rec2.bytes(), s));
     HIPCHK(launch_pack_tile_records(t->lane_groups.p, (uint32_t)t->lane_groups.n, t->lane_nstates.p, t->lane_fwdx.p, t->lane_bwd.p, t->lane_rec2.p, t->lane_chain.p,
                                     t->tile_group.p, (uint32_t)(t->tile_group.n - 1), t->tile_chain.p, s));
+    if (int rc = build_tile_schedule(t, s)) return rc;
     if (lib_opt("timing")) {
       std::vector<uint32_t> ch(t->lane_chain.n);
       HIPCHK(hipMemcpyAsync(ch.data(), t->lane_chain.p, ch.size() * 4, hipMemcpyDeviceToHost, s));
@@ -346,6 +348,10 @@
     t->lane_rec2.release();
     t->lane_chain.release();
     t->tile_chain.release();
+    t->tile_sched.release();
+    t->tile_sched_wg = 0;
+    t->h_tile_sched.clear();
+    t->h_tile_shape.clear();
   }
   t->lane_records = L.wave_slot_base + L.wave_bwd.size();
   if (L.lane_fused)
@@ -1140,7 +1146,8 @@
         HIPCHK(hipEventRecord(t->cev[q], t->cstream[q]));
         HIPCHK(hipStreamWaitEvent(s, t->cev[q], 0));
       }
-  } else if (tile_sweep && launch_tile_sweep(TZ, LA, t->tile_group.p, 0, lane_tiles, s) == hipSuccess) {
+  } else if (tile_sweep && launch_tile_sweep(TZ, LA, t->tile_group.p, 0, lane_tiles, lib_opt_off("tile_sweep_balance") ? nullptr : t->tile_sched.p,
+                                             t->tile_sched_wg, (uint32_t)(t->tile_group.n - 1), s) == hipSuccess) {
     tile_sweep_done = true;
   } else {
     if (tile_sweep) (void)hipGetLastError();
@@ -1263,6 +1270,63 @@
     if (rc) return rc;
   }
   return matrix_setup(t, &t->matrix);
+}
+int build_tile_schedule(carmel_hip_trainer* t, hipStream_t s) {
+  t->tile_sched.release();
+  t->tile_sched_wg = 0;
+  t->h_tile_sched.clear();
+  t->h_tile_shape.clear();
+  const uint32_t n_tiles = t->tile_group.n ? (uint32_t)(t->tile_group.n - 1) : 0u;
+  uint32_t n_wg = 0;
+  if (!n_tiles || tile_sweep_workgroups(n_tiles, &n_wg) != hipSuccess || !n_wg) return (void)hipGetLastError(), CARMEL_HIP_OK;
+  std::vector<uint32_t> tg(n_tiles + 1), tc(n_tiles);
+  std::vector<LaneGroup> groups(t->lane_groups.n);
+  HIPCHK(hipMemcpyAsync(tg.data(), t->tile_group.p, tg.size() * 4, hipMemcpyDeviceToHost, s));
+  HIPCHK(hipMemcpyAsync(tc.data(), t->tile_chain.p, tc.size() * 4, hipMemcpyDeviceToHost, s));
+  HIPCHK(hipMemcpyAsync(groups.data(), t->lane_groups.p, groups.size() * sizeof(LaneGroup), hipMemcpyDeviceToHost, s));
+  HIPCHK(hipStreamSynchronize(s));
+  std::vector<double> cost(n_tiles);
+  t->h_tile_shape.resize((size_t)n_tiles * 3);
+  for (uint32_t i = 0; i < n_tiles; ++i) {
+    uint32_t ml = 0;
+    for (uint32_t g = tg[i]; g < tg[i + 1] && g < groups.size(); ++g) ml = std::max(ml, groups[g].maxlen);
+    uint32_t* sh = &t->h_tile_shape[(size_t)i * 3];
+    sh[0] = tg[i + 1] - tg[i];
+    sh[1] = ml;
+    sh[2] = tc[i] ? 1u : 0u;
+    cost[i] = tile_cost(sh[0], sh[1], sh[2] != 0);
+  }
+  std::vector<uint32_t> tiles, off;
+  tile_schedule(cost, n_wg, tiles, off);
+  t->h_tile_sched = off;
+  t->h_tile_sched.insert(t->h_tile_sched.end(), tiles.begin(), tiles.end());
+  HIPCHK(t->tile_sched.upload(t->h_tile_sched, s));
+  HIPCHK(hipStreamSynchronize(s));
+  t->tile_sched_wg = n_wg;
+  return CARMEL_HIP_OK;
+}
+int carmel_hip_tile_schedule(const uint32_t* n_groups, const uint32_t* maxlen, const uint32_t* chain, uint32_t n_tiles, uint32_t n_wg,
+                             uint32_t* tiles_out, uint32_t* off_out, double* cost_out) {
+  if ((n_tiles && (!n_groups || !maxlen || !chain || !tiles_out)) || !off_out) return fail(CARMEL_HIP_ERR_ARG, "null argument");
+  std::vector<double> cost(n_tiles);
+  for (uint32_t i = 0; i < n_tiles; ++i) cost[i] = tile_cost(n_groups[i], maxlen[i], chain[i] != 0);
+  std::vector<uint32_t> tiles, off;
+  tile_schedule(cost, n_wg, tiles, off);
+  std::copy(tiles.begin(), tiles.end(), tiles_out);
+  std::copy(off.begin(), off.end(), off_out);
+  if (cost_out) std::copy(cost.begin(), cost.end(), cost_out);
+  return CARMEL_HIP_OK;
+}
+int carmel_hip_lattice_tile_schedule(carmel_hip_trainer* t, uint32_t* n_wg, uint32_t* shapes_out, uint32_t* tiles_out, uint32_t* off_out) {
+  if (!t || !n_wg) return fail(CARMEL_HIP_ERR_ARG, "null argument");
+  *n_wg = 0;
+  if (!carmel_hip_lattice_tile_sweep(t) || !t->tile_sched_wg) return CARMEL_HIP_OK;
+  *n_wg = t->tile_sched_wg;
+  const size_t n_off = (size_t)t->tile_sched_wg + 1;
+  if (shapes_out) std::copy(t->h_tile_shape.begin(), t->h_tile_shape.end(), shapes_out);
+  if (off_out) std::copy(t->h_tile_sched.begin(), t->h_tile_sched.begin() + n_off, off_out);
+  if (tiles_out) std::copy(t->h_tile_sched.begin() + n_off, t->h_tile_sched.end(), tiles_out);
+  return CARMEL_HIP_OK;
 }
 int carmel_hip_lattice_tile_sweep(carmel_hip_trainer* t) {
   if (!t || !t->have_lattices || t->unrolled || !t->lat.tile_sweep || !t->tile_group.n) return 0;
diff --git a/carmel_amd/csrc/engine.hpp b/carmel_amd/csrc/engine.hpp
--- a/carmel_amd/csrc/engine.hpp
+++ b/carmel_amd/csrc/engine.hpp
@@ -125,6 +125,9 @@
   DevBuf<uint32_t> lane_rec2;
   DevBuf<uint32_t> lane_chain;
   DevBuf<uint32_t> tile_chain;
+  DevBuf<uint32_t> tile_sched;
+  uint32_t tile_sched_wg = 0;
+  std::vector<uint32_t> h_tile_sched, h_tile_shape;
   DevBuf<uint2_t> lane_fwd;
   DevBuf<TransBucket> t_buckets;
   DevBuf<uint64_t> t_tile_base;
@@ -189,6 +192,7 @@
 
 extern "C" int mstep_args(carmel_hip_trainer* t, int use_counts, int save_old, MstepArgs& M);
 extern "C" void trans_args(carmel_hip_trainer* t, TransArgs& T);
+extern "C" int build_tile_schedule(carmel_hip_trainer* t, hipStream_t s);
 bool exchange_is_sharded(const ExchangePlan* xp);
 extern "C" int publish_u64(carmel_hip_trainer* t, const unsigned long long* dev, hipStream_t s);
 extern "C" int fetch_u64(carmel_hip_trainer* t, const unsigned long long* dev, unsigned long long* out, hipStream_t s, bool published);
diff --git a/carmel_amd/csrc/kernels.hpp b/carmel_amd/csrc/kernels.hpp
--- a/carmel_amd/csrc/kernels.hpp
+++ b/carmel_amd/csrc/kernels.hpp
@@ -169,8 +169,9 @@
 hipError_t launch_trans_w_bucket(const TransArgs& T, hipStream_t stream);
 hipError_t launch_trans_w_bucket_range(const TransArgs& T, uint32_t first, uint32_t count, hipStream_t stream);
 hipError_t launch_trans_c_bucket_range(const TransArgs& T, uint32_t first, uint32_t count, hipStream_t stream);
+hipError_t tile_sweep_workgroups(uint32_t tile_count, uint32_t* n_wg);
 hipError_t launch_tile_sweep(const TransArgs& T, const LaneArgs& A, const uint32_t* tile_group, uint32_t tile_first, uint32_t tile_count,
-                             hipStream_t stream);
+                             const uint32_t* sched, uint32_t sched_wg, uint32_t sched_tiles, hipStream_t stream);
 hipError_t launch_pack_tile_records(const LaneGroup* groups, uint32_t n_groups, const uint32_t* lane_nstates, const uint32_t* fwdx,
                                     const uint32_t* bwd, uint32_t* out, uint32_t* chain, const uint32_t* tile_group, uint32_t n_tiles,
                                     uint32_t* tile_chain, hipStream_t stream);
diff --git a/carmel_amd/csrc/lattice_gpu.hip b/carmel_amd/csrc/lattice_gpu.hip
--- a/carmel_amd/csrc/lattice_gpu.hip
+++ b/carmel_amd/csrc/lattice_gpu.hip
@@ -1252,6 +1252,7 @@
     HIPCHK(hipMemsetAsync(t->lane_rec2.p, 0, n_rec * 4, s));
     HIPCHK(launch_pack_tile_records(t->lane_groups.p, (uint32_t)t->lane_groups.n, t->lane_nstates.p, t->lane_fwdx.p, t->lane_bwd.p, t->lane_rec2.p, t->lane_chain.p,
                                     t->tile_group.p, (uint32_t)(t->tile_group.n - 1), t->tile_chain.p, s));
+    if (int rc = build_tile_schedule(t, s)) return rc;
     if (lib_opt("timing")) {
       std::vector<uint32_t> ch(t->lane_chain.n);
       HIPCHK(hipMemcpyAsync(ch.data(), t->lane_chain.p, ch.size() * 4, hipMemcpyDeviceToHost, s));
@@ -1264,6 +1265,10 @@
     t->lane_rec2.release();
     t->lane_chain.release();
     t->tile_chain.release();
+    t->tile_sched.release();
+    t->tile_sched_wg = 0;
+    t->h_tile_sched.clear();
+    t->h_tile_shape.clear();
   }
   lap("record streams");
   {
diff --git a/carmel_amd/csrc/options.cpp b/carmel_amd/csrc/options.cpp
--- a/carmel_amd/csrc/options.cpp
+++ b/carmel_amd/csrc/options.cpp
@@ -11,7 +11,7 @@
     "timing",
     "lane_states", "tile_sweep", "lane_fused", "transpose", "lane_chunks", "lane_window", "lane_window_min", "wave_ring", "wave_min_width",
     "gpu_build", "wave_gather", "wave_xc", "tile_gather", "device_tables", "trans_scatter", "trans_runs", "lane_fused_kernel",
-    "tile_sweep_kernel", "mailbox", "poison", "lane_trace", "exchange_sparse", "mstep_wide",
+    "tile_sweep_kernel", "tile_sweep_balance", "mailbox", "poison", "lane_trace", "exchange_sparse", "mstep_wide",
     "dense", "unrolled", "unrolled_ragged",
     "gibbs_chains", "gibbs_own_cap", "gibbs_workgroup", "gibbs_clk", "gibbs_reg", "gibbs_lane", "forest_sweep", "forest_ldswalk", "forest_multi",
     "forest_nohash", "forest_trace", "forest_exact_host", "forest_exact_clk", "forest_logdomain", "forest_gcol", "forest_gather",
diff --git a/carmel_amd/csrc/tile_schedule.hpp b/carmel_amd/csrc/tile_schedule.hpp
--- /dev/null
+++ b/carmel_amd/csrc/tile_schedule.hpp
@@ -0,0 +1,130 @@
+#pragma once
+#include <algorithm>
+#include <cstdint>
+#include <vector>
+
+namespace carmel_hip {
+
+constexpr double TILE_COST_FIXED = 8750.0;
+constexpr double TILE_COST_ROW = 137.0;
+constexpr double TILE_COST_GROUP = 1800.0;
+constexpr double TILE_COST_MOVER = 10100.0;
+constexpr double TILE_COST_MOVER_SWEEP = 3000.0;
+constexpr double TILE_COST_MOVER_ROUND = 700.0;
+constexpr uint32_t TILE_SCHED_SLOTS = 8;
+constexpr uint32_t TILE_SCHED_SWEEPERS = 4;
+
+inline uint32_t tile_cost_rounds(uint32_t n_groups, bool chain) {
+  const uint32_t r = (n_groups + TILE_SCHED_SWEEPERS - 1) / TILE_SCHED_SWEEPERS;
+  return chain && r > 1 ? r - 1 : std::max(r, 1u);
+}
+inline double tile_cost(uint32_t n_groups, uint32_t maxlen, bool chain) {
+  const uint32_t rounds = tile_cost_rounds(n_groups, chain);
+  const double sweep = rounds * (TILE_COST_ROW * maxlen + TILE_COST_GROUP);
+  const double mover = TILE_COST_MOVER + (chain && n_groups > TILE_SCHED_SWEEPERS ? TILE_COST_MOVER_SWEEP : 0.0) + TILE_COST_MOVER_ROUND * (rounds - 1);
+  return TILE_COST_FIXED + std::max(sweep, mover);
+}
+
+inline uint32_t tile_sched_slot_wgs(uint32_t n_wg, uint32_t s) { return s < n_wg ? (n_wg - s + TILE_SCHED_SLOTS - 1) / TILE_SCHED_SLOTS : 0; }
+
+inline double tile_sched_slot_max(const std::vector<double>& cost, uint32_t lo, uint32_t hi, uint32_t W, std::vector<double>& scratch) {
+  if (hi <= lo) return 0.0;
+  if (!W) return 1e300;
+  scratch.assign(W, 0.0);
+  for (uint32_t i = lo; i < hi; ++i) scratch[(i - lo) % W] += cost[i];
+  return *std::max_element(scratch.begin(), scratch.end());
+}
+
+inline void tile_schedule(const std::vector<double>& cost, uint32_t n_wg, std::vector<uint32_t>& tiles, std::vector<uint32_t>& off) {
+  const uint32_t n = (uint32_t)cost.size();
+  tiles.assign(n, 0u);
+  off.assign((size_t)n_wg + 1, 0u);
+  if (!n_wg) return;
+  const uint32_t S = std::min(TILE_SCHED_SLOTS, n_wg);
+  std::vector<uint32_t> cut(S + 1, 0u), W(S);
+  double total = 0.0;
+  for (double c : cost) total += c;
+  {
+    uint32_t wsum = 0, i = 0;
+    double run = 0.0;
+    for (uint32_t s = 0; s < S; ++s) {
+      W[s] = tile_sched_slot_wgs(n_wg, s);
+      wsum += W[s];
+      const double share = total * wsum / n_wg;
+      while (i < n && run + 0.5 * cost[i] <= share) run += cost[i++];
+      cut[s + 1] = s + 1 == S ? n : i;
+    }
+  }
+  std::vector<double> scratch, smax(S);
+  for (uint32_t s = 0; s < S; ++s) smax[s] = tile_sched_slot_max(cost, cut[s], cut[s + 1], W[s], scratch);
+  std::vector<uint32_t> eq(S + 1);
+  const uint32_t per = (n + S - 1) / S;
+  for (uint32_t s = 0; s <= S; ++s) eq[s] = (uint32_t)std::min<uint64_t>((uint64_t)s * per, n);
+  const bool one_each = per <= *std::min_element(W.begin(), W.end());
+  for (uint32_t iter = 0; !one_each && iter < 64 * S; ++iter) {
+    const uint32_t s = (uint32_t)(std::max_element(smax.begin(), smax.end()) - smax.begin());
+    double best = smax[s];
+    int dir = 0;
+    double best_a = 0, best_b = 0;
+    if (s > 0 && cut[s + 1] - cut[s] > 1) {
+      const double a = tile_sched_slot_max(cost, cut[s - 1], cut[s] + 1, W[s - 1], scratch);
+      const double b = tile_sched_slot_max(cost, cut[s] + 1, cut[s + 1], W[s], scratch);
+      if (std::max(a, b) < best) best = std::max(a, b), dir = -1, best_a = a, best_b = b;
+    }
+    if (s + 1 < S && cut[s + 1] - cut[s] > 1) {
+      const double a = tile_sched_slot_max(cost, cut[s], cut[s + 1] - 1, W[s], scratch);
+      const double b = tile_sched_slot_max(cost, cut[s + 1] - 1, cut[s + 2], W[s + 1], scratch);
+      if (std::max(a, b) < best) best = std::max(a, b), dir = 1, best_a = a, best_b = b;
+    }
+    if (!dir) break;
+    if (dir < 0) {
+      ++cut[s];
+      smax[s - 1] = best_a;
+      smax[s] = best_b;
+    } else {
+      --cut[s + 1];
+      smax[s] = best_a;
+      smax[s + 1] = best_b;
+    }
+  }
+  if (!one_each) {
+    std::vector<uint32_t> g(S + 1, 0u), g_best;
+    double lo_b = total / n_wg, hi_b = *std::max_element(smax.begin(), smax.end());
+    for (int it = 0; it < 40 && hi_b - lo_b > 1e-6 * hi_b; ++it) {
+      const double bound = 0.5 * (lo_b + hi_b);
+      uint32_t i = 0;
+      for (uint32_t s = 0; s < S; ++s) {
+        scratch.assign(W[s], 0.0);
+        const uint32_t first = i;
+        while (i < n && scratch[(i - first) % W[s]] + cost[i] <= bound) scratch[(i - first) % W[s]] += cost[i], ++i;
+        g[s + 1] = i;
+      }
+      if (i == n)
+        hi_b = bound, g_best = g;
+      else
+        lo_b = bound;
+    }
+    if (!g_best.empty()) {
+      double g_max = 0.0;
+      for (uint32_t s = 0; s < S; ++s) g_max = std::max(g_max, tile_sched_slot_max(cost, g_best[s], g_best[s + 1], W[s], scratch));
+      if (g_max < *std::max_element(smax.begin(), smax.end())) {
+        cut = g_best;
+        for (uint32_t s = 0; s < S; ++s) smax[s] = tile_sched_slot_max(cost, cut[s], cut[s + 1], W[s], scratch);
+      }
+    }
+  }
+  {
+    double eq_max = 0.0;
+    for (uint32_t s = 0; s < S; ++s) eq_max = std::max(eq_max, tile_sched_slot_max(cost, eq[s], eq[s + 1], W[s], scratch));
+    if (one_each || eq_max < *std::max_element(smax.begin(), smax.end())) cut = eq;
+  }
+  std::vector<uint32_t> cnt((size_t)n_wg, 0u);
+  for (uint32_t s = 0; s < S; ++s)
+    for (uint32_t i = cut[s]; i < cut[s + 1]; ++i) ++cnt[s + TILE_SCHED_SLOTS * ((i - cut[s]) % W[s])];
+  for (uint32_t b = 0; b < n_wg; ++b) off[b + 1] = off[b] + cnt[b];
+  std::vector<uint32_t> at(off.begin(), off.end() - 1);
+  for (uint32_t s = 0; s < S; ++s)
+    for (uint32_t i = cut[s]; i < cut[s + 1]; ++i) tiles[at[s + TILE_SCHED_SLOTS * ((i - cut[s]) % W[s])]++] = i;
+}
+
+}
diff --git a/carmel_amd/csrc/tile_sweep.hip b/carmel_amd/csrc/tile_sweep.hip
--- a/carmel_amd/csrc/tile_sweep.hip
+++ b/carmel_amd/csrc/tile_sweep.hip
@@ -385,11 +385,37 @@
   uint64_t i0, i1;
   bool ok;
 };
-__device__ __forceinline__ TileWalk tile_walk_at(const TransArgs& T, const LaneArgs& A, const uint32_t* __restrict__ tile_group, uint32_t vidx,
-                                                 bool ok, uint32_t z) {
+struct TileSched {
+  const uint32_t* tiles;
+  uint32_t pos, end;
+  uint32_t ahead;
+};
+__device__ __forceinline__ TileSched tile_sched_begin(const uint32_t* __restrict__ sched) {
+  TileSched S;
+  S.tiles = sched ? sched + gridDim.x + 1 : nullptr;
+  S.pos = sched ? sched[blockIdx.x] : blockIdx.x;
+  S.end = sched ? sched[blockIdx.x + 1] : 0u;
+  S.ahead = 0;
+  return S;
+}
+__device__ __forceinline__ void tile_sched_request(TileSched& S) {
+  if (S.tiles) S.ahead = S.tiles[min(S.pos + 3, S.end - 1)];
+}
+__device__ __forceinline__ void tile_sched_advance(TileSched& S) { S.pos += S.tiles ? 1u : gridDim.x; }
+__device__ __forceinline__ TileWalk tile_walk_at(const TransArgs& T, const LaneArgs& A, const uint32_t* __restrict__ tile_group, const TileSched& S,
+                                                 uint32_t k, bool ok, uint32_t z, bool arrived) {
   TileWalk w;
-  const uint32_t tloc = xcd_chunked(vidx, T.tile_count);
-  w.ok = ok && tloc < T.tile_count && vidx / 8 < (T.tile_count + 7) / 8;
+  uint32_t tloc;
+  bool in;
+  if (S.tiles) {
+    in = S.pos + k < S.end;
+    tloc = arrived ? S.ahead : S.tiles[in ? S.pos + k : 0u];
+  } else {
+    const uint32_t v = S.pos + k * gridDim.x;
+    tloc = xcd_chunked(v, T.tile_count);
+    in = tloc < T.tile_count && v / 8 < (T.tile_count + 7) / 8;
+  }
+  w.ok = ok && in;
   w.tile = T.tile_first + (w.ok ? tloc : 0u);
   w.i0 = T.tile_base[w.tile + z];
   w.i1 = T.tile_base[w.tile + 1 + z];
@@ -412,21 +438,23 @@
   return w;
 }
 template <bool SCAT>
-__global__ __launch_bounds__(TILE_SWEEP_THREADS) void tile_sweep_kernel(TransArgs T, LaneArgs A, const uint32_t* __restrict__ tile_group) {
+__global__ __launch_bounds__(TILE_SWEEP_THREADS) void tile_sweep_kernel(TransArgs T, LaneArgs A, const uint32_t* __restrict__ tile_group,
+                                                                       const uint32_t* __restrict__ sched) {
   extern __shared__ __attribute__((aligned(16))) double lds[];
   constexpr int NM = TILE_SWEEP_MOVERS, KT = (int)(TILE_SWEEP_TILE / NM), NW = (TILE_SWEEP_THREADS - NM) / 64;
   uint32_t* const recs = (uint32_t*)(lds + TILE_SWEEP_TILE);
   double* const alpha = lds + TILE_SWEEP_TILE + TILE_SWEEP_TILE / 2;
   const int lane = threadIdx.x & 63;
   const uint32_t wv = __builtin_amdgcn_readfirstlane(threadIdx.x >> 6);
-  uint32_t vidx = blockIdx.x;
   const uint32_t z = ts_zero();
   for (uint32_t i = blockIdx.x * TILE_SWEEP_THREADS + threadIdx.x; i < T.n_zero; i += gridDim.x * TILE_SWEEP_THREADS) T.counts[T.zero_list[i]] = 0.0;
-  TileWalk cur = tile_walk_at(T, A, tile_group, vidx, true, z);
+  TileSched S = tile_sched_begin(sched);
+  TileWalk cur = tile_walk_at(T, A, tile_group, S, 0, true, z, false);
   if (!cur.ok) return;
   cur = ts_uniform(cur);
-  TileWalk nxt = ts_uniform(tile_walk_at(T, A, tile_group, vidx + gridDim.x, true, z));
-  TileWalk nn_raw = tile_walk_at(T, A, tile_group, vidx + 2 * gridDim.x, nxt.ok, z);
+  TileWalk nxt = ts_uniform(tile_walk_at(T, A, tile_group, S, 1, true, z, false));
+  tile_sched_request(S);
+  TileWalk nn_raw = tile_walk_at(T, A, tile_group, S, 2, nxt.ok, z, false);
   if (wv >= (uint32_t)NW) {
     const uint32_t m = threadIdx.x - (uint32_t)(TILE_SWEEP_THREADS - NM);
     TileIn in;
@@ -452,6 +480,8 @@
         if (m + k * NM < cur.ni) lds[in.pos[k]] = in.v[k];
       }
       __syncthreads();
+      uint32_t m1 = 0, m2 = 0;
+      if (A.trace) m1 = m2 = (uint32_t)__builtin_readcyclecounter();
       if (nxt.ok) tile_request<SCAT>(T, A, nxt.tile, nxt.i0, nxt.ni, m, in);
       {
         const LaneGroup gm = ts_uniform(gm_raw);
@@ -466,6 +496,7 @@
           const uint32_t off = (uint32_t)(gm.stream_base - (uint64_t)cur.tile * TILE_SWEEP_TILE) + lane;
           const double lp = tile_chain_sweep(gm, lm_cur, cm >> 8, lane, alpha + (size_t)gm.spill_row * 64 + lane, lds + off);
           if ((uint32_t)lane < gm.n_lanes) A.pair_logprob[lm_cur.pair] = lp;
+          if (A.trace) m2 = (uint32_t)__builtin_readcyclecounter();
         }
       }
       uint32_t dst[KT];
@@ -475,6 +506,8 @@
 #pragma unroll
         for (int k = 0; k < KT; ++k) dst[k] = sp[k * NM];
       }
+      if (A.trace && lane == 0)
+        A.trace[(size_t)cur.tile * 16 + 12 + mw] = ((unsigned long long)(m2 - m1) << 32) | ((uint32_t)__builtin_readcyclecounter() - m1);
       __syncthreads();
       tile_exp_in_place(lds);
       __syncthreads();
@@ -486,10 +519,11 @@
       }
       if (!nxt.ok) break;
       __syncthreads();
-      vidx += gridDim.x;
+      tile_sched_advance(S);
       cur = nxt;
       nxt = ts_uniform(nn_raw);
-      nn_raw = tile_walk_at(T, A, tile_group, vidx + 2 * gridDim.x, nxt.ok, z);
+      nn_raw = tile_walk_at(T, A, tile_group, S, 2, nxt.ok, z, true);
+      tile_sched_request(S);
     }
   } else {
     constexpr int KR = (int)(TILE_SWEEP_TILE / 4 / (TILE_SWEEP_THREADS - NM));
@@ -564,14 +598,17 @@
         o[2] = t2 - t1;
         o[4] = ((unsigned long long)(cur.g1 - cur.g0) << 32) | cur.ni;
         o[5] = ((unsigned long long)__builtin_amdgcn_s_getreg((4 << 0) | (0 << 6) | (31 << 11)) << 32) | g.maxlen;
+        o[6] = blockIdx.x;
+        o[7] = ((unsigned long long)cur.chain << 32) | A.groups[cur.g0].maxlen;
       }
       if (!nxt.ok) break;
       __syncthreads();
       if (A.trace && threadIdx.x == 0) A.trace[(size_t)cur.tile * 16 + 3] = __builtin_readcyclecounter() - t2;
-      vidx += gridDim.x;
+      tile_sched_advance(S);
       cur = nxt;
       nxt = ts_uniform(nn_raw);
-      nn_raw = tile_walk_at(T, A, tile_group, vidx + 2 * gridDim.x, nxt.ok, z);
+      nn_raw = tile_walk_at(T, A, tile_group, S, 2, nxt.ok, z, true);
+      tile_sched_request(S);
       g = ts_uniform(g_n);
       L = L_n;
       chain = ts_sc(chain_n);
@@ -579,32 +616,39 @@
   }
 }
 #define TRANS_SET_LDS(K, BYTES) (void)hipFuncSetAttribute((const void*)K, hipFuncAttributeMaxDynamicSharedMemorySize, BYTES)
-hipError_t launch_tile_sweep(const TransArgs& T0, const LaneArgs& A, const uint32_t* tile_group, uint32_t tile_first, uint32_t tile_count,
-                             hipStream_t stream) {
-  if (!T0.n_buckets || !tile_count) return hipSuccess;
-  if (T0.tile != TILE_SWEEP_TILE || !A.pre_weights || !A.rec2 || !A.chain || !A.tile_chain) return hipErrorInvalidValue;
-  if (T0.slack_bytes < TILE_SWEEP_TILE * sizeof(double)) return hipErrorInvalidValue;
+hipError_t tile_sweep_workgroups(uint32_t tile_count, uint32_t* n_wg) {
   int dev = 0;
   if (hipGetDevice(&dev) != hipSuccess || dev < 0 || dev >= 64) return hipErrorInvalidDevice;
   static int dev_cus[64] = {0};
-  const int lds = (int)TILE_SWEEP_LDS;
   if (!dev_cus[dev]) {
-    if (hipFuncSetAttribute((const void*)tile_sweep_kernel<false>, hipFuncAttributeMaxDynamicSharedMemorySize, lds) != hipSuccess ||
-        hipFuncSetAttribute((const void*)tile_sweep_kernel<true>, hipFuncAttributeMaxDynamicSharedMemorySize, lds) != hipSuccess)
+    if (hipFuncSetAttribute((const void*)tile_sweep_kernel<false>, hipFuncAttributeMaxDynamicSharedMemorySize, (int)TILE_SWEEP_LDS) != hipSuccess ||
+        hipFuncSetAttribute((const void*)tile_sweep_kernel<true>, hipFuncAttributeMaxDynamicSharedMemorySize, (int)TILE_SWEEP_LDS) != hipSuccess)
       return hipErrorInvalidValue;
     hipDeviceProp_t prop;
     if (hipGetDeviceProperties(&prop, dev) != hipSuccess) return hipErrorInvalidDevice;
     __atomic_store_n(&dev_cus[dev], prop.multiProcessorCount > 8 ? prop.multiProcessorCount / 8 * 8 : 8, __ATOMIC_RELEASE);
   }
   const int n_cu = __atomic_load_n(&dev_cus[dev], __ATOMIC_ACQUIRE);
+  *n_wg = std::min<uint32_t>((uint32_t)n_cu, (tile_count + 7) / 8 * 8);
+  return hipSuccess;
+}
+hipError_t launch_tile_sweep(const TransArgs& T0, const LaneArgs& A, const uint32_t* tile_group, uint32_t tile_first, uint32_t tile_count,
+                             const uint32_t* sched, uint32_t sched_wg, uint32_t sched_tiles, hipStream_t stream) {
+  if (!T0.n_buckets || !tile_count) return hipSuccess;
+  if (T0.tile != TILE_SWEEP_TILE || !A.pre_weights || !A.rec2 || !A.chain || !A.tile_chain) return hipErrorInvalidValue;
+  if (T0.slack_bytes < TILE_SWEEP_TILE * sizeof(double)) return hipErrorInvalidValue;
+  uint32_t n_wg = 0;
+  if (hipError_t e = tile_sweep_workgroups(tile_count, &n_wg)) return e;
+  if (tile_first || tile_count != sched_tiles || sched_wg != n_wg) sched = nullptr;
+  const int lds = (int)TILE_SWEEP_LDS;
   TransArgs T = T0;
   T.tile_first = tile_first;
   T.tile_count = tile_count;
-  const dim3 g8(std::min<uint32_t>((uint32_t)n_cu, (tile_count + 7) / 8 * 8));
+  const dim3 g8(n_wg);
   if ((T.scatter & 3u) == 3u && T.use_runs)
-    hipLaunchKernelGGL((tile_sweep_kernel<true>), g8, dim3(TILE_SWEEP_THREADS), lds, stream, T, A, tile_group);
+    hipLaunchKernelGGL((tile_sweep_kernel<true>), g8, dim3(TILE_SWEEP_THREADS), lds, stream, T, A, tile_group, sched);
   else if (!(T.scatter & 3u))
-    hipLaunchKernelGGL((tile_sweep_kernel<false>), g8, dim3(TILE_SWEEP_THREADS), lds, stream, T, A, tile_group);
+    hipLaunchKernelGGL((tile_sweep_kernel<false>), g8, dim3(TILE_SWEEP_THREADS), lds, stream, T, A, tile_group, sched);
   else
     return hipErrorInvalidValue;
   return hipGetLastError();
diff --git a/carmel_amd/trainer.py b/carmel_amd/trainer.py
--- a/carmel_amd/trainer.py
+++ b/carmel_amd/trainer.py
@@ -168,6 +168,15 @@
     @property
     def tile_sweep_tiles(self):
         return lib.carmel_hip_lattice_tile_sweep(self.h)
+
+    def tile_schedule(self):
+        n_wg, n = C.c_uint32(0), self.tile_sweep_tiles
+        u32p = C.POINTER(C.c_uint32)
+        if lib.carmel_hip_lattice_tile_schedule(self.h, C.byref(n_wg), None, None, None) or not n_wg.value:
+            return None
+        shapes, tiles, off = np.zeros((n, 3), np.uint32), np.zeros(n, np.uint32), np.zeros(n_wg.value + 1, np.uint32)
+        lib.carmel_hip_lattice_tile_schedule(self.h, C.byref(n_wg), *(a.ctypes.data_as(u32p) for a in (shapes, tiles, off)))
+        return n_wg.value, shapes, tiles, off
 
     @property
     def fused_lane_tiles(self):
diff --git a/include/carmel_hip.h b/include/carmel_hip.h
--- a/include/carmel_hip.h
+++ b/include/carmel_hip.h
@@ -57,6 +57,9 @@
 
 int carmel_hip_debug_lattice_fingerprint(carmel_hip_trainer* t, uint64_t* out16);
 int carmel_hip_lattice_tile_sweep(carmel_hip_trainer* t);
+int carmel_hip_tile_schedule(const uint32_t* n_groups, const uint32_t* maxlen, const uint32_t* chain, uint32_t n_tiles, uint32_t n_wg,
+                             uint32_t* tiles_out, uint32_t* off_out, double* cost_out);
+int carmel_hip_lattice_tile_schedule(carmel_hip_trainer* t, uint32_t* n_wg, uint32_t* shapes_out, uint32_t* tiles_out, uint32_t* off_out);
 int carmel_hip_lattice_fused_lanes(carmel_hip_trainer* t);
 int carmel_hip_lattice_weight_source(carmel_hip_trainer* t);
 int carmel_hip_lattice_layout(carmel_hip_trainer* t);
```

Result: no change. 53.41 billion arc-updates/s (median of 3 runs) (+0.6%).
